# keillernogueira/dynamic-rs-segmentation

Hardware: AMD Instinct MI355X
Metric: training patches/sec dilated_grsl_rate8 64x64x5 (higher is better)
Workload: dtype f32; 1 GPU; dilated_grsl_rate8 (Dilated8Pooling) training step, single_fixed 64x64, 5-band synthetic 2048x2048 tile, global batch 128 (crop+augment+normalise, fwd, loss, bwd, momentum, confusion); global_batch=128, patch=64, bands=5, classes=6, parallelism=dp1, sync_bn=True, rccl_ranks_observed=1

## Files before the change

dynamic-rs-segmentation_amd/_lib.py:

```python
import ctypes as C
import os

_HERE = os.path.dirname(os.path.abspath(__file__))
LIB_PATH = os.path.join(_HERE, "libdrs_hip.so")
DEV_LIB_PATH = os.path.join(_HERE, "libdrs_hip_dev.so")

_p, _i, _f, _d = C.c_void_p, C.c_int, C.c_float, C.c_double
_sz, _u64 = C.c_size_t, C.c_ulonglong

SIGNATURES = {
    "drs_conv_mtile": (_i, [_i]),
    "drs_conv_forward": (_i, [_p, _i, _i, _i, _i, _i, _p, _p, _i, _i, _i, _i, _i, _p, _i, _i, _i, _p, _p]),
    "drs_conv_workspace_floats": (_sz, [_i]),
    "drs_conv_halo_skip": (_i, [_i, _i, _i, _i, _i, _i, _i]),
    "drs_conv_executed_ksteps": (_i, [_i, _i, _i, _i, _i, _i, _i, _p, _p]),
    "drs_conv_forward_ws": (_i, [_p, _i, _i, _i, _i, _i, _p, _p, _i, _i, _i, _i, _i, _p, _i, _i, _i, _p, _p, _sz, _p]),
    "drs_conv_wgrad_splits": (_i, [_i, _i, _i, _i, _i]),
    "drs_conv_wgrad": (_i, [_p, _i, _i, _i, _i, _i, _p, _i, _i, _i, _i, _i, _i, _i, _i, _i, _p, _p, _p]),
    "drs_filter_flip_transpose": (_i, [_p, _p, _i, _i, _i, _p]),
    "drs_filter_pad_cin": (_i, [_p, _p, _i, _i, _i, _i, _p]),
    "drs_split_conv_mtile": (_i, [_i]),
    "drs_split_terms": (_i, [_p, _sz, _i, _p, _p]),
    "drs_filter_split": (_i, [_p, _i, _i, _i, _i, _i, _p, _p, _p]),
    "drs_conv_forward_split": (_i, [_p, _i, _i, _i, _i, _i, _p, _p, _i, _i, _i, _i, _i, _p, _i, _i, _i, _p, _i, _p]),
    "drs_conv_wgrad_split_splits": (_i, [_i, _i, _i, _i, _i, _i, _i]),
    "drs_conv_wgrad_split": (_i, [_p, _i, _i, _i, _i, _i, _p, _i, _i, _i, _i, _i, _i, _i, _i, _i, _p, _p, _i, _p]),
    "drs_colsum_scratch_doubles": (_i, [_i]),
    "drs_stats_reduce": (_i, [_p, _i, _i, _p, _p, _p]),
    "drs_stats_reduce_means": (_i, [_p, _i, _i, _d, _p, _p, _p]),
    "drs_conv_stats_reduce": (_i, [_p, _i, _i, _i, _p, _p, _p]),
    "drs_conv_stats_finish": (_i, [_p, _i, _i, _i, _d, _p, _p, _p, _d, _i, _p, _p]),
    "drs_bn_finish": (_i, [_p, _d, _i, _p, _p, _p, _d, _i, _p]),
    "drs_bn_eval_coeffs": (_i, [_p, _p, _i, _p, _p]),
    "drs_bn_act_pool_forward": (_i, [_p, _i, _i, _i, _p, _f, _i, _p, _i, _i, _i, _p, _p]),
    "drs_bn_finish_act_pool_forward": (_i, [_p, _d, _p, _p, _p, _d, _i, _p, _i, _i, _i, _f, _i, _p, _i, _i, _i, _p, _p]),
    "drs_bn_act_pool_forward_terms": (_i, [_p, _i, _i, _i, _p, _f, _i, _p, _i, _i, _i, _p, _p, _i, _p]),
    "drs_bn_backward_rows": (_i, [_i, _i, _i, _i]),
    "drs_bn_backward_reduce": (_i, [_p, _i, _i, _p, _p, _i, _i, _i, _p, _f, _i, _p, _p, _p]),
    "drs_bn_backward_apply": (_i, [_p, _p, _i, _i, _i, _p, _p, _d, _p, _i, _i, _i, _p]),
    "drs_bn_backward_apply_means": (_i, [_p, _p, _i, _i, _i, _p, _p, _p, _i, _i, _i, _p]),
    "drs_bn_backward_apply_terms": (_i, [_p, _p, _i, _i, _i, _p, _p, _d, _p, _i, _i, _i, _p, _i, _p]),
    "drs_avg_pool_forward": (_i, [_p, _i, _i, _i, _i, _p, _i, _i, _i, _p]),
    "drs_avg_pool_backward": (_i, [_p, _i, _i, _i, _i, _i, _i, _p, _p]),
    "drs_se_forward": (_i, [_p, _i, _i, _i, _i, _p, _p, _p, _p, _p, _p, _p, _p, _i, _i, _i, _p]),
    "drs_se_backward": (_i, [_p, _i, _i, _p, _p, _p, _p, _p, _p, _i, _i, _i, _i, _p, _p, _p, _p, _p, _p, _p]),
    "drs_se_core_sums_scratch_doubles": (_i, [_i]),
    "drs_se_core_sums": (_i, [_p, _i, _i, _p, _i, _p, _p, _p]),
    "drs_se_gate": (_i, [_p, _d, _i, _i, _p, _p, _p, _p, _p, _p, _p, _p]),
    "drs_se_scale_const": (_i, [_p, _i, _i, _i, _p, _p, _i, _i, _i, _p]),
    "drs_classifier_rows": (_i, [_i, _i]),
    "drs_classifier_loss": (_i, [_p, _i, _i, _i, _i, _i, _i, _i, _p, _p, _p, _p, _p, _f, _p, _p, _p, _i, _i, _p, _p, _p,
                                 _p, _p]),
    "drs_classifier_loss_weighted": (_i, [_p, _i, _i, _i, _i, _i, _i, _i, _p, _p, _p, _p, _p, _f, _p, _p, _p, _p, _i, _i, _p, _p,
                                          _p, _p, _p]),
    "drs_classifier_loss_focal": (_i, [_p, _i, _i, _i, _i, _i, _i, _i, _p, _p, _p, _p, _p, _f, _p, _f, _p, _p, _p, _i, _i, _p, _p,
                                       _p, _p, _p]),
    "drs_label_histogram": (_i, [_p, _sz, _i, _i, _p, _p]),
    "drs_reliability_histogram": (_i, [_p, _p, _p, _sz, _i, _i, _p, _p]),
    "drs_temperature_scratch_doubles": (_sz, [_sz]),
    "drs_temperature_stats": (_i, [_p, _p, _p, _sz, _i, _i, _i, _d, _p, _p, _p]),
    "drs_rows_reduce_f32": (_i, [_p, _i, _i, _p, _p, _p]),
    "drs_sum_f64": (_i, [_p, _i, _p, _p]),
    "drs_l2_loss": (_i, [_p, _sz, _p, _p, _p]),
    "drs_momentum_update": (_i, [_p, _p, _p, _sz, _sz, _f, _f, _f, _f, _p]),
    "drs_confusion": (_i, [_p, _p, _p, _sz, _i, _i, _p, _p]),
    "drs_crop_normalize": (_i, [_p, _i, _p, _p, _p, _p, _p, _i, _p, _p, _p, _p, _p, _u64, _i, _p, _p, _i, _i, _i, _i, _p, _p,
                                _p, _i, _i, _p]),
    "drs_crop_normalize_scaled": (_i, [_p, _i, _p, _p, _p, _p, _p, _i, _i, _p, _p, _p, _p, _p, _p, _u64, _i, _p, _p, _i, _i, _i, _i,
                                       _p, _p, _p, _i, _i, _p]),
    "drs_stitch_accumulate": (_i, [_p, _p, _p, _i, _i, _i, _i, _i, _i, _i, _p]),
    "drs_stitch_finalize": (_i, [_p, _p, _i, _i, _i, _p, _p]),
    "drs_stitch_finalize_scores": (_i, [_p, _p, _i, _i, _i, _i, _p, _p, _p, _p, _p]),
    "drs_stitch_finalize_scores_t": (_i, [_p, _p, _i, _i, _i, _i, _f, _p, _p, _p, _p, _p]),
    "drs_tile_place": (_i, [_p, _p, _p, _i, _i, _i, _i, _p, _i, _p]),
    "drs_crop_dihedral": (_i, [_p, _i, _p, _p, _p, _i, _i, _p, _i, _p, _p, _i, _i, _i, _i, _p, _p]),
    "drs_tile_place_dihedral": (_i, [_p, _p, _p, _i, _i, _i, _i, _p, _i, _i, _p]),
    "drs_crop_resampled": (_i, [_p, _i, _p, _p, _p, _i, _i, _p, _i, _i, _i, _p, _p, _i, _i, _i, _i, _p, _p]),
    "drs_resample_accumulate": (_i, [_p, _p, _i, _i, _i, _i, _i, _i, _p, _p]),
    "drs_softmax_accumulate": (_i, [_p, _p, _i, _i, _i, _p, _p]),
    "drs_scale_f64": (_i, [_p, _i, _d, _p]),
    "drs_net_create": (_i, [C.c_char_p, _i, _i, _f, _i, _i, _i, _f, C.POINTER(_p)]),
    "drs_net_destroy": (None, [_p]),
    "drs_net_num_buffers": (_i, [_p]),
    "drs_net_buffer_info": (_i, [_p, _i, C.c_char_p, _i, C.POINTER(_sz), C.POINTER(_i)]),
    "drs_net_bind": (_i, [_p, C.c_char_p, _p, _sz]),
    "drs_net_buffer": (_i, [_p, C.c_char_p, C.POINTER(_p), C.POINTER(_sz)]),
    "drs_net_layout": (_i, [_p, C.POINTER(_sz), C.POINTER(_sz), C.POINTER(_sz), C.POINTER(_i), C.POINTER(_i), C.POINTER(_i)]),
    "drs_net_layer_info": (_i, [_p, _i, C.c_char_p, _i, C.POINTER(_i), C.c_char_p, C.c_char_p, _i, C.POINTER(_i), C.POINTER(_i)]),
    "drs_net_info": (_i, [_p, C.c_char_p, _i, C.POINTER(_f), C.POINTER(_i), C.c_char_p, _i, C.POINTER(_i), C.POINTER(_i)]),
    "drs_net_receptive_field": (_i, [_p, C.POINTER(_i), C.POINTER(_i)]),
    "drs_net_receptive_field_gated": (_i, [_p, C.POINTER(_i), C.POINTER(_i)]),
    "drs_net_se_info": (_i, [_p, _i, C.c_char_p, _i, C.POINTER(_i), C.POINTER(_i), C.POINTER(_i)]),
    "drs_net_type_name": (_i, [_i, C.c_char_p, _i, C.POINTER(_i)]),
    "drs_net_num_variables": (_i, [_p]),
    "drs_net_variable_info": (_i, [_p, _i, C.c_char_p, _i, C.POINTER(_sz), C.POINTER(_sz), C.POINTER(_i), C.POINTER(_i)]),
    "drs_params_get": (_i, [_p, C.c_char_p, C.c_char_p, _p, _sz, _p]),
    "drs_params_set": (_i, [_p, C.c_char_p, C.c_char_p, _p, _sz, _p]),
    "drs_grad_buffer": (_i, [_p, C.POINTER(_p), C.POINTER(_sz)]),
    "drs_net_global_step": (C.c_longlong, [_p, C.c_longlong]),
    "drs_net_learning_rate": (_f, [_p, _f]),
    "drs_net_set_comm": (_i, [_p, _i, _i, _p, _p, _p]),
    "drs_rccl_bind_library": (_i, [C.c_char_p]),
    "drs_rccl_available": (_i, []),
    "drs_rccl_form": (_i, []),
    "drs_rccl_unique_id": (_i, [_p]),
    "drs_rccl_comm_create": (_i, [_i, _i, _p, C.POINTER(_p)]),
    "drs_rccl_comm_destroy": (_i, [_p]),
    "drs_rccl_all_reduce": (_i, [_p, _p, C.c_size_t, _i, _p]),
    "drs_net_set_rccl": (_i, [_p, _i, _i, _p, _p, _p]),
    "drs_train_step": (_i, [_p, _i, _i, _f, _i, _d, _p]),
    "drs_forward": (_i, [_p, _i, _i, _i, _i, _p]),
    "drs_apply_update": (_i, [_p, _f, _p]),
    "drs_forward_staged": (_i, [_p, _i, _i, _i, _p, _i, _i, _p]),
    "drs_net_se_gate_finish": (_i, [_p, _i, _d, _p]),
    "drs_net_set_two_streams": (_i, [_p, _i]),
    "drs_net_set_class_weights": (_i, [_p, _p, _i]),
    "drs_net_get_class_weights": (_i, [_p, _p, _i, C.POINTER(_i)]),
    "drs_net_set_focal_gamma": (_i, [_p, _f]),
    "drs_net_get_focal_gamma": (_i, [_p, C.POINTER(_f)]),
    "drs_net_timing": (_i, [_p, _i]),
    "drs_net_num_timing_kinds": (_i, []),
    "drs_net_timing_summary": (_i, [_p, _i, C.c_char_p, _i, C.POINTER(_i), C.POINTER(_d), C.POINTER(_d)]),
}
ALLREDUCE_FN = C.CFUNCTYPE(_i, _p, _p, _sz, _i, _i, _p)
WAIT_FN = C.CFUNCTYPE(_i, _p, _i, _p)
WANT_LOGITS, WITH_LABELS, USE_ACC_MASK, USE_LOSS_MASK, NO_UPDATE = 1, 2, 4, 8, 16


DEV_SIGNATURES = {
    "drs_debug_skip_taps": (_i, [_i]), "drs_debug_conv_variant": (_i, [_i]), "drs_debug_conv_wide192": (_i, [_i]),
    "drs_debug_conv_splitk": (_i, [_i]), "drs_debug_conv_hybrid": (_i, [_i]), "drs_debug_conv_sk_order": (_i, [_i]), "drs_debug_conv_prio": (_i, [_i]),
    "drs_debug_conv_sk_geometry": (_i, [_i, _i, _i, _p]), "drs_debug_conv_trace": (_i, [_p]), "drs_debug_conv_lpt": (_i, [_i]), "drs_debug_conv_order": (_i, [_i] * 7 + [_p, _i]),
    "drs_debug_conv_image_tiles": (_i, [_i]), "drs_debug_conv_order_image": (_i, [_i] * 7 + [_p, _i]),
    "drs_debug_wgrad_variant": (_i, [_i]), "drs_debug_wgrad_seg": (_i, [_i]), "drs_debug_wgrad_balance": (_i, [_i]), "drs_debug_wgrad_target": (_i, [_i]),
    "drs_debug_wgrad_target_big": (_i, [_i]), "drs_debug_wgrad_len": (_i, [_i]), "drs_debug_wgrad_minchunks": (_i, [_i]), "drs_debug_wgrad_model": (_i, [_i]), "drs_debug_wgrad_ablate": (_i, [_i]), "drs_debug_wgrad_prio": (_i, [_i]), "drs_debug_cls_variant": (_i, [_i]), "drs_debug_slide_blocks": (_i, [_i]), "drs_debug_slide_minrows": (_i, [_i]), "drs_debug_slide_rowpad": (_i, [_i]), "drs_debug_chain_mode": (_i, [_i]), "drs_debug_jitter": (_i, [C.c_ulonglong]), "drs_debug_wg_stream_prio": (_i, [_i]), "drs_debug_reductions_on_chain": (_i, [_i]), "drs_debug_wgrad_schedule": (_i, [_i, _i, _i]), "drs_debug_variant": (_i, [_i]),
    "drs_debug_wgrad_cut": (_i, [_i] * 7 + [_p, _i, _p, _p]),
}


class DrsError(RuntimeError):
    pass


_lib = None
_dev = None


def _open(path, signatures):
    if not os.path.isfile(path):
        raise DrsError("HIP library not built: %s is missing (run dynamic-rs-segmentation_amd/csrc/build.sh "
                       "or __graft_entry__.build()); there is no CPU fallback" % path)
    import torch
    lib = C.CDLL(path)
    for name, (res, args) in signatures.items():
        fn = getattr(lib, name)
        fn.restype = res
        fn.argtypes = args
    return lib


def load():
    global _lib
    if _lib is None:
        _lib = _open(LIB_PATH, SIGNATURES)
    return _lib


class _Dev(object):

    def __init__(self, lib):
        self.lib = lib

    def __getattr__(self, name):
        return getattr(self.lib, name)

    def load(self):
        return self.lib

    def call(self, name, *args):
        rc = getattr(self.lib, name)(*args)
        if rc != 0:
            raise DrsError("%s -> %s" % (name, _STATUS.get(rc, rc)))

    def query(self, name, *args):
        return getattr(self.lib, name)(*args)


def dev():
    global _dev
    if _dev is None:
        sig = dict(SIGNATURES)
        sig.update(DEV_SIGNATURES)
        _dev = _Dev(_open(DEV_LIB_PATH, sig))
    return _dev


_STATUS = {1: "DRS_ERR_ARG (rejected argument)", 2: "DRS_ERR_HIP (launch failed)"}


def call(name, *args):
    rc = getattr(load(), name)(*args)
    if rc != 0:
        raise DrsError("%s -> %s" % (name, _STATUS.get(rc, rc)))


def query(name, *args):
    return getattr(load(), name)(*args)
```

dynamic-rs-segmentation_amd/csrc/conv_mfma.hip:

```cpp
#include "drs_common.hpp"
#include <algorithm>
#include <cstdlib>
#include <map>
#include <mutex>
#include <numeric>
#include <tuple>
#include <vector>

namespace {

constexpr int BK = 32;
constexpr int LDA = BK + 4;

struct ConvArgs {
  const float* in; int S, P, ld_in, coff_in;
  int M;
  const float* w;
  const float* bias;
  float* out; int ld_out, coff_out;
  float* stats;
  int k, rate, pad, Cin, Cout;
  int accumulate;
  int skip_halo;
  float rcpS, rcpSS;
  float* sk_slab;
  int sk_W, sk_nks, sk_U;
  int sk_T, sk_tiles, sk_G, sk_order;
  int prio;
  int lpt_T, lpt_ta, lpt_tb, lpt_P;
  int img_g;
  const int* img_order;
#ifdef DRS_DEV
  unsigned long long* trace;
#endif
};

__device__ __forceinline__ void set_prio_by_progress(int done, int total, int& quarter, int mode = 1) {
  const int q = __builtin_amdgcn_readfirstlane((done * 4) / total);
  if (q == quarter) return;
  quarter = q;
  if (mode == 2) {
    if (q <= 0) __builtin_amdgcn_s_setprio(2);
    else if (q == 1) __builtin_amdgcn_s_setprio(1);
    else __builtin_amdgcn_s_setprio(0);
    return;
  }
  if (q <= 0) __builtin_amdgcn_s_setprio(3);
  else if (q == 1) __builtin_amdgcn_s_setprio(2);
  else if (q == 2) __builtin_amdgcn_s_setprio(1);
  else __builtin_amdgcn_s_setprio(0);
}

__host__ __device__ __forceinline__ int lpt_tile(int wg, int T, int ta, int tb, int P, int ntn) {
  const int per = P * T * ntn, nI = tb - ta, nE = T - nI;
  const int chunk = wg / per;
  int wl = wg - chunk * per, p, t;
  if (wl < P * nI * ntn) {
    p = wl / (nI * ntn);
    wl -= p * nI * ntn;
    t = ta + wl / ntn;
  } else {
    wl -= P * nI * ntn;
    p = wl / (nE * ntn);
    wl -= p * nE * ntn;
    const int e = wl / ntn;
    t = e < ta ? e : tb + (e - ta);
  }
  return ((chunk * P + p) * T + t) * ntn + wl % ntn;
}

__host__ __device__ __forceinline__ int sk_first_unit(int w, int U, int W) { return (int)((long long)w * U / W); }
__host__ __device__ __forceinline__ int sk_owner(int x, int U, int W) { return (int)((((long long)x + 1) * W - 1) / U); }

template <int BM, int BN, int WM, int WN, bool MAP = false>
__device__ __forceinline__ void conv_epilogue(const ConvArgs& a, f32x16 (&acc)[BM / WM / 32][BN / WN / 32], float* scratch, int m0, int n0,
                                              int pix0 = 0, int pcs = 30) {
  constexpr int WTM = BM / WM, WTN = BN / WN;
  constexpr int TM = WTM / 32, TN = WTN / 32;
  const int t = threadIdx.x;
  const int lane = t & 63, wave = t >> 6;
  const int li = lane & 31, h = lane >> 5;
  const int wm = wave / WN, wn = wave % WN;
  const int pcm = (1 << pcs) - 1, S2 = a.S * a.S;
  const int lane_rl = wm * WTM + 4 * h;
  const int lane_pix = MAP ? pix0 + (lane_rl >> pcs) * S2 + (lane_rl & pcm) : 0;
  float bv[TN];
#pragma unroll
  for (int ni = 0; ni < TN; ++ni) {
    const int col = n0 + wn * WTN + ni * 32 + li;
    bv[ni] = a.bias ? a.bias[col] : 0.f;
#pragma unroll
    for (int mi = 0; mi < TM; ++mi) {
#pragma unroll
      for (int r = 0; r < 16; ++r) {
        const int crl = mi * 32 + (r & 3) + 8 * (r >> 2);
        const int row = MAP ? lane_pix + __builtin_amdgcn_readfirstlane((crl >> pcs) * S2 + (crl & pcm)) : m0 + lane_rl + crl;
        if (row < a.M) {
          float v = acc[mi][ni][r] + bv[ni];
          float* dst = a.out + (size_t)row * a.ld_out + a.coff_out + col;
          if (a.accumulate) v += *dst;
          *dst = v;
        }
      }
    }
  }
  if (a.stats) {
    const int rem = a.M - m0;
    tile_column_stats<TN, WM, BN>(
        scratch, t, wm, h == 0, (float)(rem < BM ? rem : BM), [&](int ni) { return wn * WTN + ni * 32 + li; },
        [](float s) { return s + __shfl_xor(s, 32); },
        [&](int ni, auto f) {
#pragma unroll
          for (int mi = 0; mi < TM; ++mi)
#pragma unroll
            for (int r = 0; r < 16; ++r)
              if (m0 + wm * WTM + mi * 32 + (r & 3) + 8 * (r >> 2) + 4 * h < a.M) f(acc[mi][ni][r] + bv[ni]);
        },
        a.stats + ((size_t)(m0 / BM) * a.Cout + n0) * 2);
  }
}

template <int BM, int BN, int WM, int WN, bool PACK = false>
__global__ __launch_bounds__(256, (BM == 256 || BN == 128) ? 3 : 1) void conv_igemm_kernel(const ConvArgs a) {
  static_assert(WM * WN == 4, "4 waves");
  constexpr int LDB = BN + 4;
  constexpr int WTM = BM / WM, WTN = BN / WN;
  constexpr int TM = WTM / 32, TN = WTN / 32;
  constexpr int NA = BM / 32;
  constexpr int NB = BN / 32;
  constexpr int BROWS = 256 / (BN / 4);

  __shared__ __attribute__((aligned(16))) float lds[BM * LDA + BK * LDB];
  float* As = lds;
  float* Bs = lds + BM * LDA;

  const int t = threadIdx.x;
  const int lane = t & 63, wave = t >> 6;
  const int li = lane & 31, h = lane >> 5;
  const int wm = wave / WN, wn = wave % WN;

  const int ntn = a.Cout / BN;
  const int nblk = gridDim.x;
  const int tile = xcd_remap(blockIdx.x, nblk);
  const int m0 = (tile / ntn) * BM;
  const int n0 = (tile % ntn) * BN;

  const int Sp = a.S + 2 * a.P;
  uint32_t offA[NA];
#pragma unroll
  for (int i = 0; i < NA; ++i) {
    int p = m0 + (t >> 3) + 32 * i;
    p = p < a.M ? p : a.M - 1;
    offA[i] = (padded_pixel_off(p, a.S, a.P, a.ld_in, a.rcpS, a.rcpSS, -a.pad, -a.pad) + (uint32_t)(a.coff_in + (PACK ? 0 : (t & 7) * 4))) * 4u;
  }
  const int brow = t / (BN / 4), bcol = (t % (BN / 4)) * 4;
  uint32_t offB[NB];
#pragma unroll
  for (int i = 0; i < NB; ++i) offB[i] = (uint32_t)((brow + BROWS * i) * a.Cout + n0 + bcol) * 4u;

  f32x16 acc[TM][TN];
#pragma unroll
  for (int mi = 0; mi < TM; ++mi)
#pragma unroll
    for (int ni = 0; ni < TN; ++ni)
#pragma unroll
      for (int r = 0; r < 16; ++r) acc[mi][ni][r] = 0.f;

  const int cpt = a.Cin / BK;
  int u_lo, u_hi;
  live_tap_rows(m0, BM, a.M, a.S, a.k, a.rate, a.pad, a.rcpS, a.rcpSS, u_lo, u_hi);
  if (PACK || !a.skip_halo) { u_lo = 0; u_hi = a.k; }
  u_lo = __builtin_amdgcn_readfirstlane(u_lo);
  u_hi = __builtin_amdgcn_readfirstlane(u_hi);
  const int nks = PACK ? (a.k * a.k * a.Cin + BK - 1) / BK : (u_hi - u_lo) * a.k * cpt;
  const char* wlive = reinterpret_cast<const char*>(a.w + (size_t)u_lo * a.k * a.Cin * a.Cout);
  const char* inb = reinterpret_cast<const char*>(a.in);
  f32x4 ra[NA], rb[NB];
  int lu = u_lo, lv = 0, lc = 0;

  auto gload = [&](int ks) {
    if (PACK) {
      const int kidx = ks * BK + (t & 7) * 4;
      int tap = kidx / a.Cin;
      const int c = kidx - tap * a.Cin;
      tap = tap < a.k * a.k ? tap : a.k * a.k - 1;
      const int u = tap / a.k, v = tap - u * a.k;
      const uint32_t soff = (uint32_t)((u * a.rate * Sp + v * a.rate) * a.ld_in + c) * 4u;
#pragma unroll
      for (int i = 0; i < NA; ++i) ra[i] = *reinterpret_cast<const f32x4*>(inb + (offA[i] + soff));
    } else {
      const char* ab = inb + (size_t)(uint32_t)((lu * a.rate * Sp + lv * a.rate) * a.ld_in + lc * BK) * 4u;
#pragma unroll
      for (int i = 0; i < NA; ++i) { uint32_t o = offA[i]; asm volatile("" : "+v"(o)); ra[i] = *reinterpret_cast<const f32x4*>(ab + o); }
    }
    const char* wb = wlive + (size_t)(uint32_t)((PACK ? ks : ((lu - u_lo) * a.k + lv) * cpt + lc) * BK) * (uint32_t)a.Cout * 4u;
#pragma unroll
    for (int i = 0; i < NB; ++i) { uint32_t o = offB[i]; asm volatile("" : "+v"(o)); rb[i] = *reinterpret_cast<const f32x4*>(wb + o); }
    if (!PACK) { if (++lv == a.k) { lv = 0; if (++lu == u_hi) { lu = u_lo; ++lc; } } }
  };
  auto lstore = [&]() {
#pragma unroll
    for (int i = 0; i < NA; ++i) *reinterpret_cast<f32x4*>(&As[((t >> 3) + 32 * i) * LDA + (t & 7) * 4]) = ra[i];
#pragma unroll
    for (int i = 0; i < NB; ++i) *reinterpret_cast<f32x4*>(&Bs[(brow + BROWS * i) * LDB + bcol]) = rb[i];
  };

  gload(0);
  lstore();
  __syncthreads();
  const int arow = wm * WTM + li, bcolw = wn * WTN + li;
  for (int ks = 0; ks < nks; ++ks) {
    if (ks + 1 < nks) gload(ks + 1);
    {
      constexpr int NST = BK / 2;
      f32x4 af[2][TM];
      float bf[2][TN];
#pragma unroll
      for (int mi = 0; mi < TM; ++mi) af[0][mi] = *reinterpret_cast<const f32x4*>(&As[(arow + mi * 32) * LDA + h * 4]);
#pragma unroll
      for (int ni = 0; ni < TN; ++ni) bf[0][ni] = Bs[(h * 4) * LDB + bcolw + ni * 32];
#pragma unroll
      for (int st = 0; st < NST; ++st) {
        const int e = st & 3;
        if (st + 1 < NST) {
          const int q1 = (st + 1) >> 2, e1 = (st + 1) & 3;
#pragma unroll
          for (int ni = 0; ni < TN; ++ni) bf[(st + 1) & 1][ni] = Bs[(q1 * 8 + h * 4 + e1) * LDB + bcolw + ni * 32];
          if (e1 == 0) {
#pragma unroll
            for (int mi = 0; mi < TM; ++mi) af[q1 & 1][mi] = *reinterpret_cast<const f32x4*>(&As[(arow + mi * 32) * LDA + q1 * 8 + h * 4]);
            __builtin_amdgcn_sched_group_barrier(0x100, TN + TM, 0);
          } else {
            __builtin_amdgcn_sched_group_barrier(0x100, TN, 0);
          }
        }
#pragma unroll
        for (int mi = 0; mi < TM; ++mi)
#pragma unroll
          for (int ni = 0; ni < TN; ++ni)
            acc[mi][ni] = __builtin_amdgcn_mfma_f32_32x32x2f32(af[(st >> 2) & 1][mi][e], bf[st & 1][ni], acc[mi][ni], 0, 0, 0);
        __builtin_amdgcn_sched_group_barrier(0x8, TM * TN, 0);
      }
    }
    __syncthreads();
    if (ks + 1 < nks) { lstore(); __syncthreads(); }
  }

  conv_epilogue<BM, BN, WM, WN>(a, acc, lds, m0, n0);
}

template <int BM, int BN, int WM, int WN, bool SK>
__global__ __launch_bounds__(256, 3) void conv_dma_kernel(const ConvArgs a) {
#if defined(__HIP_DEVICE_COMPILE__)
  static_assert(WM * WN == 4 && BM == 128, "4 waves, 128-pixel tiles");
  constexpr int WTM = BM / WM, WTN = BN / WN;
  constexpr int TM = WTM / 32, TN = WTN / 32;
  constexpr int HK = 16;
  constexpr int ASTAGE = BM * HK, STAGE = ASTAGE + HK * BN;
  constexpr int IA = (BM / 16) / 4;
  constexpr int BQ = BN / 4;
  constexpr int IB = HK * BQ / 64 / 4;
  static_assert(IA >= 1 && IB >= 1 && IB * 4 * 64 == HK * BQ, "tile / wave layout");

  __shared__ __attribute__((aligned(1024))) float lds[2 * STAGE];

  const int t = threadIdx.x;
  const int lane = t & 63, wave = __builtin_amdgcn_readfirstlane(t >> 6);
  const int li = lane & 31, h = lane >> 5;
  const int wm = wave / WN, wn = wave % WN;
  const int ntn = a.Cout / BN;
  const int wg = xcd_remap(blockIdx.x, gridDim.x);
#ifdef DRS_DEV
  if (a.trace && t == 0) a.trace[2 * blockIdx.x] = __builtin_amdgcn_s_memrealtime();
#endif
  const int Sp = a.S + 2 * a.P;
  const int cpt = a.Cin / BK;
  typedef __attribute__((address_space(3))) void* lds_ptr;
  const __amdgpu_buffer_rsrc_t rsrc_in = __builtin_amdgcn_make_buffer_rsrc(const_cast<float*>(a.in), 0, 0xffffffff, 0x00020000);
  const __amdgpu_buffer_rsrc_t rsrc_w = __builtin_amdgcn_make_buffer_rsrc(const_cast<float*>(a.w), 0, 0xffffffff, 0x00020000);
  const int arow = wm * WTM + li, bcolw = wn * WTN + li;
  const int sw = (li >> 2) & 3;

  int u = 0, u_end = 1, rng = 0, dp_next = 0;
  bool dp_first = false;
  if (SK) {
    const int jb = (int)(((long long)wg * a.sk_W + a.sk_G - 1) / a.sk_G), je = (int)(((long long)(wg + 1) * a.sk_W + a.sk_G - 1) / a.sk_G);
    rng = __builtin_amdgcn_readfirstlane(jb);
    u = u_end = 0;
    if (je > jb) {
      u = __builtin_amdgcn_readfirstlane(sk_first_unit(jb, a.sk_U, a.sk_W));
      u_end = __builtin_amdgcn_readfirstlane(sk_first_unit(jb + 1, a.sk_U, a.sk_W));
    }
    dp_next = a.sk_T + wg;
    if (u >= u_end && dp_next >= a.sk_tiles) return;
    dp_first = a.sk_order == 1 || (a.sk_order == 2 && ((blockIdx.x >> 8) & 1));
  }
  const int img_g = SK ? 0 : a.img_g;
  int tile0 = wg;
  if (!SK && img_g) {
    const int mpos = wg / ntn;
    tile0 = __builtin_amdgcn_readfirstlane(a.img_order[mpos] * ntn + (wg - mpos * ntn));
  } else if (!SK && a.lpt_T) {
    tile0 = __builtin_amdgcn_readfirstlane(lpt_tile(wg, a.lpt_T, a.lpt_ta, a.lpt_tb, a.lpt_P, ntn));
  }
  bool first_seg = true;
  int quart = -1, done = 0, total = 1;
  if (a.prio == 3) __builtin_amdgcn_s_setprio(3);
  if (SK && a.prio) total = (u_end - u) + (dp_next < a.sk_tiles ? ((a.sk_tiles - 1 - dp_next) / a.sk_G + 1) * a.sk_nks : 0);
  for (;;) {
    int tile = tile0, kb = 0, ke = 0;
    bool in_range = false;
    if (SK) {
      in_range = u < u_end && !(dp_first && dp_next < a.sk_tiles);
      if (in_range) {
        tile = u / a.sk_nks;
        kb = u - tile * a.sk_nks;
        ke = kb + (u_end - u);
        ke = ke < a.sk_nks ? ke : a.sk_nks;
      } else {
        tile = dp_next;
        dp_next += a.sk_G;
        kb = 0;
        ke = a.sk_nks;
      }
    }
    const int m0 = (tile / ntn) * BM;
    const int n0 = (tile % ntn) * BN;
    int ty = 0, tx0 = 0, timg0 = 0;
    if (!SK && img_g) {
      const int grp = image_tile_pos(tile / ntn, a.S, img_g, ty, tx0);
      ty = __builtin_amdgcn_readfirstlane(ty);
      tx0 = __builtin_amdgcn_readfirstlane(tx0);
      timg0 = __builtin_amdgcn_readfirstlane(grp << img_g);
    }

    uint32_t offA[IA], offB[IB];
#pragma unroll
    for (int i = 0; i < IA; ++i) {
      const int r = (wave + 4 * i) * 16 + (lane >> 2);
      uint32_t pix;
      if (!SK && img_g) {
        const int pcs = 7 - img_g;
        pix = (uint32_t)(((timg0 + (r >> pcs)) * Sp + ty + a.P - a.pad) * Sp + (tx0 + (r & ((1 << pcs) - 1)) + a.P - a.pad)) * (uint32_t)a.ld_in;
      } else {
        int p = m0 + r;
        p = p < a.M ? p : a.M - 1;
        pix = padded_pixel_off(p, a.S, a.P, a.ld_in, a.rcpS, a.rcpSS, -a.pad, -a.pad);
      }
      offA[i] = (pix + (uint32_t)a.coff_in) * 4u + (uint32_t)(((lane & 3) ^ ((lane >> 4) & 3)) * 16);
    }
#pragma unroll
    for (int i = 0; i < IB; ++i) {
      const int f = 64 * (wave + 4 * i) + lane;
      offB[i] = (uint32_t)(((f / BQ) * a.Cout + n0 + (f % BQ) * 4)) * 4u;
    }

    f32x16 acc[TM][TN];
#pragma unroll
    for (int mi = 0; mi < TM; ++mi)
#pragma unroll
      for (int ni = 0; ni < TN; ++ni)
#pragma unroll
        for (int r = 0; r < 16; ++r) acc[mi][ni][r] = 0.f;

    int u_lo, u_hi, v_lo = 0, v_hi = a.k;
    if (!SK && img_g) live_taps_image_tile(ty, tx0, 128 >> img_g, a.S, a.k, a.rate, a.pad, u_lo, u_hi, v_lo, v_hi);
    else live_tap_rows(m0, BM, a.M, a.S, a.k, a.rate, a.pad, a.rcpS, a.rcpSS, u_lo, u_hi);
    if (!a.skip_halo || SK) { u_lo = 0; u_hi = a.k; v_lo = 0; v_hi = a.k; }
    u_lo = __builtin_amdgcn_readfirstlane(u_lo);
    u_hi = __builtin_amdgcn_readfirstlane(u_hi);
    v_lo = __builtin_amdgcn_readfirstlane(v_lo);
    v_hi = __builtin_amdgcn_readfirstlane(v_hi);
    const int nks = (u_hi - u_lo) * (v_hi - v_lo) * cpt;
    if (!SK) ke = nks;
    const uint32_t wlive_off = (uint32_t)(u_lo * a.k * a.Cin * a.Cout) * 4u;
    int lu = u_lo, lv = v_lo, lc = 0;
    if (SK && kb) {
      const int per_chunk = (u_hi - u_lo) * a.k;
      lc = kb / per_chunk;
      const int rem = kb - lc * per_chunk;
      lu = u_lo + rem / a.k;
      lv = rem - (rem / a.k) * a.k;
      lc = __builtin_amdgcn_readfirstlane(lc); lu = __builtin_amdgcn_readfirstlane(lu); lv = __builtin_amdgcn_readfirstlane(lv);
    }

    auto issue = [&](int half, int stage) {
      float* sa = lds + stage * STAGE;
      float* sb = sa + ASTAGE;
      const uint32_t ao = (uint32_t)((lu * a.rate * Sp + lv * a.rate) * a.ld_in + lc * BK + half * HK) * 4u;
      const uint32_t wo = wlive_off + (uint32_t)((((lu - u_lo) * a.k + lv) * cpt + lc) * BK + half * HK) * (uint32_t)a.Cout * 4u;
#pragma unroll
      for (int i = 0; i < IA; ++i)
        __builtin_amdgcn_raw_ptr_buffer_load_lds(rsrc_in, (lds_ptr)(sa + (wave + 4 * i) * 256), 16, (int)offA[i], (int)ao, 0, 0);
#pragma unroll
      for (int i = 0; i < IB; ++i)
        __builtin_amdgcn_raw_ptr_buffer_load_lds(rsrc_w, (lds_ptr)(sb + (wave + 4 * i) * 256), 16, (int)offB[i], (int)wo, 0, 0);
    };
    auto next_kstep = [&]() { if (++lv == v_hi) { lv = v_lo; if (++lu == u_hi) { lu = u_lo; ++lc; } } };

    auto compute = [&](int stage) {
      const float* As = lds + stage * STAGE;
      const float* Bs = As + ASTAGE;
      constexpr int NST = HK / 2;
      f32x4 af[2][TM];
      float bf[2][TN];
#pragma unroll
      for (int mi = 0; mi < TM; ++mi) af[0][mi] = *reinterpret_cast<const f32x4*>(&As[(arow + mi * 32) * HK + ((h ^ sw) * 4)]);
#pragma unroll
      for (int ni = 0; ni < TN; ++ni) bf[0][ni] = Bs[(h * 4) * BN + bcolw + ni * 32];
#pragma unroll
      for (int st = 0; st < NST; ++st) {
        const int e = st & 3;
        if (st + 1 < NST) {
          const int q1 = (st + 1) >> 2, e1 = (st + 1) & 3;
#pragma unroll
          for (int ni = 0; ni < TN; ++ni) bf[(st + 1) & 1][ni] = Bs[(q1 * 8 + h * 4 + e1) * BN + bcolw + ni * 32];
          if (e1 == 0) {
#pragma unroll
            for (int mi = 0; mi < TM; ++mi)
              af[q1 & 1][mi] = *reinterpret_cast<const f32x4*>(&As[(arow + mi * 32) * HK + (((2 * q1 + h) ^ sw) * 4)]);
            __builtin_amdgcn_sched_group_barrier(0x100, TN + TM, 0);
          } else {
            __builtin_amdgcn_sched_group_barrier(0x100, TN, 0);
          }
        }
#pragma unroll
        for (int mi = 0; mi < TM; ++mi)
#pragma unroll
          for (int ni = 0; ni < TN; ++ni)
            acc[mi][ni] = __builtin_amdgcn_mfma_f32_32x32x2f32(af[(st >> 2) & 1][mi][e], bf[st & 1][ni], acc[mi][ni], 0, 0, 0);
        __builtin_amdgcn_sched_group_barrier(0x8, TM * TN, 0);
      }
    };

    issue(0, 0);
    asm volatile("s_waitcnt vmcnt(0)" ::: "memory");
    __syncthreads();
    if (!SK && a.prio) total = nks;
    for (int ks = kb; ks < ke; ++ks) {
      if (a.prio == 1) set_prio_by_progress(SK ? done + (ks - kb) : ks, total, quart);
      issue(1, 1);
      compute(0);
      asm volatile("s_waitcnt vmcnt(0)" ::: "memory");
      __syncthreads();
      next_kstep();
      if (ks + 1 < ke) issue(0, 0);
      compute(1);
      asm volatile("s_waitcnt vmcnt(0)" ::: "memory");
      __syncthreads();
    }
    if (!SK) {
      conv_epilogue<BM, BN, WM, WN, true>(a, acc, lds, m0, n0, img_g ? (timg0 * a.S + ty) * a.S + tx0 : m0, img_g ? 7 - img_g : 30);
    } else if (kb == 0 && ke == nks) {
      conv_epilogue<BM, BN, WM, WN>(a, acc, lds, m0, n0);
    } else {
      float* piece = a.sk_slab + (size_t)(2 * rng + (first_seg ? 0 : 1)) * (BM * BN) + (size_t)wave * (TM * TN * 16 * 64) + lane * 4;
#pragma unroll
      for (int mi = 0; mi < TM; ++mi)
#pragma unroll
        for (int ni = 0; ni < TN; ++ni)
#pragma unroll
          for (int q = 0; q < 4; ++q)
            *reinterpret_cast<f32x4*>(piece + ((mi * TN + ni) * 4 + q) * 256) =
                f32x4{acc[mi][ni][4 * q], acc[mi][ni][4 * q + 1], acc[mi][ni][4 * q + 2], acc[mi][ni][4 * q + 3]};
    }
    if (!SK) break;
    done += ke - kb;
    if (in_range) { u += ke - kb; first_seg = false; }
    if (u >= u_end && dp_next >= a.sk_tiles) break;
    __syncthreads();
  }
#ifdef DRS_DEV
  if (a.trace && t == 0) a.trace[2 * blockIdx.x + 1] = __builtin_amdgcn_s_memrealtime();
#endif
#endif
}

template <int BM, int BN, int WM, int WN>
__global__ __launch_bounds__(256) void conv_sk_fixup_kernel(const ConvArgs a) {
  constexpr int WTM = BM / WM, WTN = BN / WN;
  constexpr int TM = WTM / 32, TN = WTN / 32;
  __shared__ float lds[2 * WM * BN];
  if (a.prio == 3) __builtin_amdgcn_s_setprio(3);
  const int tile = blockIdx.x;
  const int x0 = tile * a.sk_nks;
  const int w_first = sk_owner(x0, a.sk_U, a.sk_W), w_last = sk_owner(x0 + a.sk_nks - 1, a.sk_U, a.sk_W);
  if (w_first == w_last) return;
  const int lane = threadIdx.x & 63, wave = threadIdx.x >> 6;
  const int ntn = a.Cout / BN;
  const int m0 = (tile / ntn) * BM, n0 = (tile % ntn) * BN;
  f32x16 acc[TM][TN];
#pragma unroll
  for (int mi = 0; mi < TM; ++mi)
#pragma unroll
    for (int ni = 0; ni < TN; ++ni)
#pragma unroll
      for (int r = 0; r < 16; ++r) acc[mi][ni][r] = 0.f;
  auto piece_of = [&](int w) {
    const int slot = 2 * w + (sk_first_unit(w, a.sk_U, a.sk_W) >= x0 ? 0 : 1);
    return a.sk_slab + (size_t)slot * (BM * BN) + (size_t)wave * (TM * TN * 16 * 64) + lane * 4;
  };
  constexpr int NF = TM * TN * 4;
  int w = w_first;
  if (NF <= 16) {
    for (; w + 1 <= w_last; w += 2) {
      const float* pa = piece_of(w);
      const float* pb = piece_of(w + 1);
      f32x4 va[NF], vb[NF];
#pragma unroll
      for (int f = 0; f < NF; ++f) va[f] = *reinterpret_cast<const f32x4*>(pa + f * 256);
#pragma unroll
      for (int f = 0; f < NF; ++f) vb[f] = *reinterpret_cast<const f32x4*>(pb + f * 256);
#pragma unroll
      for (int f = 0; f < NF; ++f)
#pragma unroll
        for (int j = 0; j < 4; ++j) acc[(f >> 2) / TN][(f >> 2) % TN][4 * (f & 3) + j] += va[f][j];
#pragma unroll
      for (int f = 0; f < NF; ++f)
#pragma unroll
        for (int j = 0; j < 4; ++j) acc[(f >> 2) / TN][(f >> 2) % TN][4 * (f & 3) + j] += vb[f][j];
    }
  }
  for (; w <= w_last; ++w) {
    const float* piece = piece_of(w);
#pragma unroll
    for (int mi = 0; mi < TM; ++mi)
#pragma unroll
      for (int ni = 0; ni < TN; ++ni)
#pragma unroll
        for (int q = 0; q < 4; ++q) {
          const f32x4 v = *reinterpret_cast<const f32x4*>(piece + ((mi * TN + ni) * 4 + q) * 256);
#pragma unroll
          for (int j = 0; j < 4; ++j) acc[mi][ni][4 * q + j] += v[j];
        }
  }
  conv_epilogue<BM, BN, WM, WN>(a, acc, lds, m0, n0);
}

constexpr int WG_MAXT = 64, WG_MAXC = 8;
struct WgradPlan {
  int nclass;
  int n[WG_MAXC];
  int seg_start[WG_MAXC + 1];
  int seg_width[WG_MAXC];
  unsigned char cls[WG_MAXT];
};

struct WgradArgs {
  const float* x; int S, Px, ld_x, coff_x;
  const float* g; int Pg, ld_g, coff_g;
  int M;
  int k, rate, pad, Cin, Cout;
  float* slab;
  int chunks_per_split;
  int ntr, nto;
  int skip_halo;
  int live_cut;
  int prio;
  int ablate;
  float rcpS, rcpSS;
  WgradPlan plan;
#ifdef DRS_DEV
  unsigned long long* trace;
#endif
};

__host__ __device__ __forceinline__ int wave_uniform(int v) {
#if defined(__HIP_DEVICE_COMPILE__)
  return __builtin_amdgcn_readfirstlane(v);
#else
  return v;
#endif
}

__host__ __device__ __forceinline__ void wgrad_assign(const WgradArgs& a, int TR, int id, int& tile, int& split, int& cbeg, int& cend,
                                                      int& live_lo, int& live_hi) {
  const int nchunks_total = (a.M + 31) / 32;
  const int rows_all = a.k * a.k * a.Cin;
  int nr = 0;
  if (a.plan.nclass == 0) {
    const int ntile = a.ntr * a.nto;
    split = id / ntile;
    tile = id % ntile;
  } else {
    int j = 0;
    while (j + 1 < a.plan.nclass && id >= a.plan.seg_start[j + 1]) ++j;
    const int rel = id - a.plan.seg_start[j];
    split = (j ? a.plan.n[j - 1] : 0) + rel / a.plan.seg_width[j];
    const int pos = rel % a.plan.seg_width[j];
    const int want = pos / a.nto;
    int r = 0, seen = 0;
    for (; r < a.ntr; ++r)
      if (a.plan.cls[r] >= j) { if (seen == want) break; ++seen; }
    r = r < a.ntr ? r : a.ntr - 1;
    tile = r * a.nto + pos % a.nto;
    nr = a.plan.n[a.plan.cls[r]];
  }
  tile = wave_uniform(tile);
  split = wave_uniform(split);
  const int R0 = (tile / a.nto) * TR;
  const int rlast = (R0 + TR < rows_all ? R0 + TR : rows_all) - 1;
  int lo, hi;
  live_pixel_range(R0, rlast, a.Cin, a.k, a.rate, a.pad, a.S, a.live_cut, lo, hi);
  if (a.plan.nclass == 0) {
    cbeg = split * a.chunks_per_split;
    cend = cbeg + a.chunks_per_split;
    cend = cend < nchunks_total ? cend : nchunks_total;
  } else {
    const int S2 = a.S * a.S, lp = hi - lo;
    const int live_total = (a.M / S2) * lp;
    const int q = (live_total + nr - 1) / nr;
    auto bound = [&](int s) -> int {
      if (s <= 0) return 0;
      const long long jp = (long long)s * q;
      if (s >= nr || jp >= live_total) return nchunks_total;
      const int img = (int)jp / lp, rem = (int)jp - img * lp;
      return (img * S2 + lo + rem) >> 5;
    };
    cbeg = bound(split);
    cend = bound(split + 1);
  }
  cbeg = wave_uniform(cbeg);
  cend = wave_uniform(cend);
  if (!a.skip_halo) { lo = 0; hi = a.S * a.S; }
  live_lo = lo; live_hi = hi;
}

struct ChunkWalk {
  int c, b, r, y, x0;
  int S, S2, lo, hi, ylo;
  __device__ __forceinline__ void init(int cfirst, int S_, float rcpS, float rcpSS, int lo_, int hi_) {
    S = S_; S2 = S_ * S_; lo = lo_; hi = hi_;
    int q;
    divmod24(lo, S, rcpS, ylo, q);
    c = next_live_chunk(cfirst - 1, S2, rcpSS, lo, hi);
    divmod24(c * 32, S2, rcpSS, b, r);
    divmod24(r, S, rcpS, y, x0);
    c = __builtin_amdgcn_readfirstlane(c); b = __builtin_amdgcn_readfirstlane(b); r = __builtin_amdgcn_readfirstlane(r);
    y = __builtin_amdgcn_readfirstlane(y); x0 = __builtin_amdgcn_readfirstlane(x0); ylo = __builtin_amdgcn_readfirstlane(ylo);
  }
  __device__ __forceinline__ int advance() {
    int r1 = r + 32, b1 = b;
    if (r1 >= S2) { r1 -= S2; ++b1; }
    if ((r1 + 31 >= lo && r1 < hi) || r1 + 31 >= S2 + lo) {
      ++c; r = r1; b = b1;
      x0 += 32;
      if (x0 >= S) { x0 -= S; ++y; }
      if (y >= S) y = 0;
      return 1;
    }
    const int tb = r1 < lo ? b1 : b1 + 1;
    const int T = tb * S2 + lo, c_old = c;
    const int f = T & 31;
    c = T >> 5;
    if (f <= lo) { b = tb; r = lo - f; } else { b = tb - 1; r = S2 + lo - f; }
    if (f == 0) { y = ylo; x0 = 0; } else { x0 = S - f; y = ylo - 1; if (y < 0) y = S - 1; }
    return c - c_old;
  }
};

template <int TR, int TO, bool AFF>
__global__ __launch_bounds__(64 * (TR >= 64 ? 2 : 1) * (TO >= 64 ? 2 : 1), 3) void wgrad_kernel(const WgradArgs a) {
  constexpr int WR = TR >= 64 ? 2 : 1, WC = TO >= 64 ? 2 : 1;
  constexpr int NT = 64 * WR * WC;
  constexpr int WTR = TR / WR, WTO = TO / WC;
  constexpr int TMr = WTR / 32, TNo = WTO / 32;
  constexpr int BP = 32;
  constexpr int LDX = TR + 4, LDG = TO + 4;
  constexpr int XQ = TR / 4, GQ = TO / 4;
  constexpr int NX = BP * XQ / NT, NG = BP * GQ / NT;
  constexpr int XPS = NT / XQ, GPS = NT / GQ;

  __shared__ __attribute__((aligned(16))) float lds[BP * LDX + BP * LDG];
  __shared__ uint32_t tabx[2][BP], tabg[2][BP];
  float* Xs = lds;
  float* Gs = lds + BP * LDX;

  const int t = threadIdx.x;
  const int lane = t & 63, wave = t >> 6;
  const int li = lane & 31, h = lane >> 5;
  const int wr = wave / WC, wc = wave % WC;

  int tile, split, cbeg, cend, live_lo, live_hi;
#ifdef DRS_DEV
  if (a.trace && t == 0) {
    a.trace[2 * blockIdx.x] = __builtin_amdgcn_s_memrealtime();
    a.trace[32768 + blockIdx.x] = (unsigned long long)__builtin_amdgcn_s_getreg(63492) | ((unsigned long long)__builtin_amdgcn_s_getreg(63508) << 32);
  }
#endif
  wgrad_assign(a, TR, xcd_remap(blockIdx.x, gridDim.x), tile, split, cbeg, cend, live_lo, live_hi);
  const int R0 = (tile / a.nto) * TR;
  const int o0 = (tile % a.nto) * TO;
  const int rows_all = a.k * a.k * a.Cin;
  const int myR = R0 + (t % XQ) * 4;
  const int myRc = myR < rows_all ? myR : 0;
  const int tap = myRc / a.Cin, c0 = myRc % a.Cin;
  const int u = tap / a.k, v = tap % a.k;
  const int Sxp = a.S + 2 * a.Px, Sgp = a.S + 2 * a.Pg;
  const uint32_t xconst = (uint32_t)((u * a.rate * Sxp + v * a.rate) * a.ld_x + a.coff_x + c0) * 4u;
  const uint32_t gconst = (uint32_t)(a.coff_g + o0 + (t % GQ) * 4) * 4u;
  const int xpix = t / XQ, gpix = t / GQ;
  constexpr bool affine = AFF;
  uint32_t xoff[NX], goff[NG];
#pragma unroll
  for (int i = 0; i < NX; ++i) xoff[i] = xconst + (affine ? (uint32_t)((xpix + XPS * i) * a.ld_x) * 4u : 0u);
#pragma unroll
  for (int i = 0; i < NG; ++i) goff[i] = gconst + (affine ? (uint32_t)((gpix + GPS * i) * a.ld_g) * 4u : 0u);

  f32x16 acc[TMr][TNo];
#pragma unroll
  for (int mi = 0; mi < TMr; ++mi)
#pragma unroll
    for (int ni = 0; ni < TNo; ++ni)
#pragma unroll
      for (int r = 0; r < 16; ++r) acc[mi][ni][r] = 0.f;

  const int nchunks_total = (a.M + BP - 1) / BP;
  const int clast = (a.M & 31) ? nchunks_total - 1 : -1;
  ChunkWalk w;
  w.init(cbeg, a.S, a.rcpS, a.rcpSS, live_lo, live_hi);

  int py = 0, px = 0;
  uint32_t ox = 0, og = 0;
  const uint32_t stepx = (uint32_t)(32 * a.ld_x) * 4u, stepg = (uint32_t)(32 * a.ld_g) * 4u;
  const uint32_t rowjx = (uint32_t)((Sxp - a.S) * a.ld_x) * 4u, rowjg = (uint32_t)((Sgp - a.S) * a.ld_g) * 4u;
  const uint32_t imgjx = (uint32_t)(Sxp * (Sxp - a.S) * a.ld_x) * 4u, imgjg = (uint32_t)(Sgp * (Sgp - a.S) * a.ld_g) * 4u;
  auto pixel_from_index = [&](int p) {
    int pb, rem;
    divmod24(p < a.M ? p : a.M - 1, w.S2, a.rcpSS, pb, rem);
    divmod24(rem, a.S, a.rcpS, py, px);
    ox = (uint32_t)(((pb * Sxp + py + a.Px - a.pad) * Sxp + px + a.Px - a.pad) * a.ld_x) * 4u;
    og = (uint32_t)(((pb * Sgp + py + a.Pg) * Sgp + px + a.Pg) * a.ld_g) * 4u;
  };
  if (!affine && t < BP) pixel_from_index(w.c * BP + t);
  auto fill_tables = [&](int slot, int stepped) {
    if (affine || t >= BP || w.c >= cend) return;
    const int p = w.c * BP + t;
    if (stepped == 1 && p < a.M && a.S >= 11) {
      px += 32; ox += stepx; og += stepg;
      if (a.S >= 32) {
        if (px >= a.S) { px -= a.S; ++py; ox += rowjx; og += rowjg; }
      } else {
#pragma unroll
        for (int k = 0; k < 3; ++k) if (px >= a.S) { px -= a.S; ++py; ox += rowjx; og += rowjg; }
      }
      if (py >= a.S) { py -= a.S; ox += imgjx; og += imgjg; }
    } else if (stepped != 0) {
      pixel_from_index(p);
    }
    tabx[slot][t] = ox;
    tabg[slot][t] = og;
  };

  const char* xbase = reinterpret_cast<const char*>(a.x);
  const char* gbase = reinterpret_cast<const char*>(a.g);
  f32x4 rx[NX], rg[NG];
  uint32_t nox[NX], nog[NG];
#pragma unroll
  for (int i = 0; i < NX; ++i) nox[i] = 0u;
#pragma unroll
  for (int i = 0; i < NG; ++i) nog[i] = 0u;
  auto fetch_offsets = [&](int slot) {
    if (affine) return;
#pragma unroll
    for (int i = 0; i < NX; ++i) nox[i] = tabx[slot][xpix + XPS * i] + xoff[i];
#pragma unroll
    for (int i = 0; i < NG; ++i) nog[i] = tabg[slot][gpix + GPS * i] + goff[i];
  };
  auto gload = [&]() {
    if (affine) {
      const char* xb = xbase + (size_t)(uint32_t)(((w.b * Sxp + w.y + a.Px - a.pad) * Sxp + w.x0 + a.Px - a.pad) * a.ld_x) * 4u;
      const char* gb = gbase + (size_t)(uint32_t)(((w.b * Sgp + w.y + a.Pg) * Sgp + w.x0 + a.Pg) * a.ld_g) * 4u;
#pragma unroll
      for (int i = 0; i < NX; ++i) { uint32_t o = xoff[i]; asm volatile("" : "+v"(o)); rx[i] = *reinterpret_cast<const f32x4*>(xb + o); }
#pragma unroll
      for (int i = 0; i < NG; ++i) { uint32_t o = goff[i]; asm volatile("" : "+v"(o)); rg[i] = *reinterpret_cast<const f32x4*>(gb + o); }
    } else {
#pragma unroll
      for (int i = 0; i < NX; ++i) rx[i] = *reinterpret_cast<const f32x4*>(xbase + nox[i]);
#pragma unroll
      for (int i = 0; i < NG; ++i) rg[i] = *reinterpret_cast<const f32x4*>(gbase + nog[i]);
    }
  };
  auto lstore = [&](int chunk) {
#pragma unroll
    for (int i = 0; i < NX; ++i) *reinterpret_cast<f32x4*>(&Xs[(xpix + XPS * i) * LDX + (t % XQ) * 4]) = rx[i];
    if (!AFF && chunk == clast) {
#pragma unroll
      for (int i = 0; i < NG; ++i)
        *reinterpret_cast<f32x4*>(&Gs[(gpix + GPS * i) * LDG + (t % GQ) * 4]) =
            chunk * BP + gpix + GPS * i < a.M ? rg[i] : f32x4{0.f, 0.f, 0.f, 0.f};
    } else {
#pragma unroll
      for (int i = 0; i < NG; ++i) *reinterpret_cast<f32x4*>(&Gs[(gpix + GPS * i) * LDG + (t % GQ) * 4]) = rg[i];
    }
  };

  int cA = w.c;
  if (cA < cend) {
    fill_tables(0, 0);
    __syncthreads();
    fetch_offsets(0);
    gload();
    int stepped = w.advance();
    int cB = w.c;
    fill_tables(1, stepped);
    lstore(cA);
    __syncthreads();
    fetch_offsets(1);
    const int xr = wr * WTR + li, gc = wc * WTO + li;
    int quart = -1;
    for (int it = 0; cA < cend; ++it) {
      if (a.prio) set_prio_by_progress(cA - cbeg, cend - cbeg, quart, a.prio);
#ifdef DRS_DEV
      if (a.ablate == 2) fetch_offsets((it + 1) & 1);
#endif
      if (cB < cend) gload();
      stepped = w.advance();
      fill_tables(it & 1, stepped);
      {
        float af[2][TMr], bf[2][TNo];
#pragma unroll
        for (int mi = 0; mi < TMr; ++mi) af[0][mi] = Xs[h * LDX + xr + mi * 32];
#pragma unroll
        for (int ni = 0; ni < TNo; ++ni) bf[0][ni] = Gs[h * LDG + gc + ni * 32];
#pragma unroll
        for (int s = 0; s < BP / 2; ++s) {
          if (s + 1 < BP / 2) {
#pragma unroll
            for (int mi = 0; mi < TMr; ++mi) af[(s + 1) & 1][mi] = Xs[(2 * s + 2 + h) * LDX + xr + mi * 32];
#pragma unroll
            for (int ni = 0; ni < TNo; ++ni) bf[(s + 1) & 1][ni] = Gs[(2 * s + 2 + h) * LDG + gc + ni * 32];
            __builtin_amdgcn_sched_group_barrier(0x100, TMr + TNo, 0);
          }
#pragma unroll
          for (int mi = 0; mi < TMr; ++mi)
#pragma unroll
            for (int ni = 0; ni < TNo; ++ni)
              acc[mi][ni] = __builtin_amdgcn_mfma_f32_32x32x2f32(af[s & 1][mi], bf[s & 1][ni], acc[mi][ni], 0, 0, 0);
          __builtin_amdgcn_sched_group_barrier(0x8, TMr * TNo, 0);
        }
      }
      __syncthreads();
      fetch_offsets(it & 1);
      if (cB < cend) { lstore(cB); __syncthreads(); }
      cA = cB;
      cB = w.c;
    }
  }
  const size_t rows_total = (size_t)a.k * a.k * a.Cin;
  float* dst = a.slab + ((size_t)split * rows_total + R0) * a.Cout + o0;
#pragma unroll
  for (int mi = 0; mi < TMr; ++mi)
#pragma unroll
    for (int ni = 0; ni < TNo; ++ni)
#pragma unroll
      for (int r = 0; r < 16; ++r) {
        const int row = wr * WTR + mi * 32 + (r & 3) + 8 * (r >> 2) + 4 * h;
        const int col = wc * WTO + ni * 32 + li;
        if (R0 + row < rows_all) dst[(size_t)row * a.Cout + col] = acc[mi][ni][r];
      }
#ifdef DRS_DEV
  if (a.trace && t == 0) a.trace[2 * blockIdx.x + 1] = __builtin_amdgcn_s_memrealtime();
#endif
}

template <int TR, int TO, int MODE>
__global__ __launch_bounds__(64 * (TR >= 64 ? 2 : 1) * (TO >= 64 ? 2 : 1), 3) void wgrad_dma_kernel(const WgradArgs a) {
#if defined(__HIP_DEVICE_COMPILE__)
  constexpr int WR = TR >= 64 ? 2 : 1, WC = TO >= 64 ? 2 : 1;
  constexpr int NW = WR * WC, NT = 64 * NW;
  constexpr int WTR = TR / WR, WTO = TO / WC;
  constexpr int TMr = WTR / 32, TNo = WTO / 32;
  constexpr int BP = 32, HP = 16;
  constexpr int XQ = TR / 4, GQ = TO / 4;
  constexpr int IX = HP * XQ / 64 / NW, IG = HP * GQ / 64 / NW;
  static_assert(IX >= 1 && IG >= 1 && IX * NW * 64 == HP * XQ && IG * NW * 64 == HP * GQ, "tile / wave layout");
  constexpr int XSTAGE = HP * TR, STAGE = HP * (TR + TO);

  __shared__ __attribute__((aligned(1024))) float lds[2 * STAGE];
  __shared__ uint32_t tabx[2][BP], tabg[2][BP];

  constexpr bool AFF = MODE == 1;
  constexpr bool SEG = MODE == 2;
  const int t = threadIdx.x;
  const int lane = t & 63, wave = (AFF || SEG) ? __builtin_amdgcn_readfirstlane(t >> 6) : t >> 6;
  const int li = lane & 31, h = lane >> 5;
  const int wr = wave / WC, wc = wave % WC;

  int tile, split, cbeg, cend, live_lo, live_hi;
#ifdef DRS_DEV
  if (a.trace && t == 0) {
    a.trace[2 * blockIdx.x] = __builtin_amdgcn_s_memrealtime();
    a.trace[32768 + blockIdx.x] = (unsigned long long)__builtin_amdgcn_s_getreg(63492) | ((unsigned long long)__builtin_amdgcn_s_getreg(63508) << 32);
  }
#endif
  wgrad_assign(a, TR, xcd_remap(blockIdx.x, gridDim.x), tile, split, cbeg, cend, live_lo, live_hi);
  const int R0 = (tile / a.nto) * TR;
  const int o0 = (tile % a.nto) * TO;
  const int rows_all = a.k * a.k * a.Cin;
  const int Sxp = a.S + 2 * a.Px, Sgp = a.S + 2 * a.Pg;
  constexpr bool affine = AFF || SEG;
  const int xq = lane % XQ;
  const int myR = R0 + xq * 4;
  const int myRc = myR < rows_all ? myR : 0;
  const int tap = myRc / a.Cin, c0 = myRc % a.Cin;
  const int u = tap / a.k, v = tap % a.k;
  const uint32_t biasx = SEG ? (uint32_t)(32 * a.ld_x) * 4u : 0u, biasg = SEG ? (uint32_t)(32 * a.ld_g) * 4u : 0u;
  const uint32_t xconst = (uint32_t)((a.ablate == 1 ? 0 : (u * a.rate * Sxp + v * a.rate)) * a.ld_x + a.coff_x + c0) * 4u + biasx;
  uint32_t xoff[IX], goff[IG];
  int xpix[IX], gpix[IG];
#pragma unroll
  for (int i = 0; i < IX; ++i) {
    xpix[i] = (64 * (wave + NW * i) + lane) / XQ;
    xoff[i] = xconst + (affine ? (uint32_t)(xpix[i] * a.ld_x) * 4u : 0u);
  }
#pragma unroll
  for (int i = 0; i < IG; ++i) {
    const int f = 64 * (wave + NW * i) + lane;
    gpix[i] = f / GQ;
    goff[i] = (uint32_t)(a.coff_g + o0 + (f % GQ) * 4) * 4u + (affine ? (uint32_t)(gpix[i] * a.ld_g) * 4u : 0u) + biasg;
  }

  f32x16 acc[TMr][TNo];
#pragma unroll
  for (int mi = 0; mi < TMr; ++mi)
#pragma unroll
    for (int ni = 0; ni < TNo; ++ni)
#pragma unroll
      for (int r = 0; r < 16; ++r) acc[mi][ni][r] = 0.f;

  const int nchunks_total = (a.M + BP - 1) / BP;
  const int clast = (a.M & 31) ? nchunks_total - 1 : -1;
  ChunkWalk w;
  w.init(cbeg, a.S, a.rcpS, a.rcpSS, live_lo, live_hi);

  int py = 0, px = 0;
  uint32_t ox = 0, og = 0;
  const uint32_t stepx = (uint32_t)(32 * a.ld_x) * 4u, stepg = (uint32_t)(32 * a.ld_g) * 4u;
  const uint32_t rowjx = (uint32_t)((Sxp - a.S) * a.ld_x) * 4u, rowjg = (uint32_t)((Sgp - a.S) * a.ld_g) * 4u;
  const uint32_t imgjx = (uint32_t)(Sxp * (Sxp - a.S) * a.ld_x) * 4u, imgjg = (uint32_t)(Sgp * (Sgp - a.S) * a.ld_g) * 4u;
  auto pixel_from_index = [&](int p) {
    int pb, rem;
    divmod24(p < a.M ? p : a.M - 1, w.S2, a.rcpSS, pb, rem);
    divmod24(rem, a.S, a.rcpS, py, px);
    ox = (uint32_t)(((pb * Sxp + py + a.Px - a.pad) * Sxp + px + a.Px - a.pad) * a.ld_x) * 4u;
    og = (uint32_t)(((pb * Sgp + py + a.Pg) * Sgp + px + a.Pg) * a.ld_g) * 4u;
  };
  if (!affine && t < BP) pixel_from_index(w.c * BP + t);
  auto fill_tables = [&](int slot, int stepped) {
    if (affine || t >= BP || w.c >= cend) return;
    const int p = w.c * BP + t;
    if (stepped == 1 && p < a.M && a.S >= 11) {
      px += 32; ox += stepx; og += stepg;
      if (a.S >= 32) {
        if (px >= a.S) { px -= a.S; ++py; ox += rowjx; og += rowjg; }
      } else {
#pragma unroll
        for (int k = 0; k < 3; ++k) if (px >= a.S) { px -= a.S; ++py; ox += rowjx; og += rowjg; }
      }
      if (py >= a.S) { py -= a.S; ox += imgjx; og += imgjg; }
    } else if (stepped != 0) {
      pixel_from_index(p);
    }
    tabx[slot][t] = ox;
    tabg[slot][t] = og;
  };

  const char* xbase = reinterpret_cast<const char*>(a.x);
  const char* gbase = reinterpret_cast<const char*>(a.g);
  typedef __attribute__((address_space(3))) void* lds_ptr;
  struct Seg { int brk; int32_t jx, jg; };
  auto chunk_bases = [&](const char*& xb, const char*& gb, Seg& sg) {
    xb = xbase + (size_t)(uint32_t)(((w.b * Sxp + w.y + a.Px - a.pad) * Sxp + w.x0 + a.Px - a.pad) * a.ld_x) * 4u;
    gb = gbase + (size_t)(uint32_t)(((w.b * Sgp + w.y + a.Pg) * Sgp + w.x0 + a.Pg) * a.ld_g) * 4u;
    if (SEG) {
      xb -= biasx; gb -= biasg;
      sg.brk = a.S - w.x0;
      const bool last = w.c == clast, img_end = w.y == a.S - 1;
      sg.jx = last ? -(int32_t)biasx : (int32_t)(rowjx + (img_end ? imgjx : 0u));
      sg.jg = last ? -(int32_t)biasg : (int32_t)(rowjg + (img_end ? imgjg : 0u));
    }
  };
  struct LaneOffsets { uint32_t x[2][IX], g[2][IG]; };
  auto fetch_offsets = [&](int slot, LaneOffsets& o) {
    if (affine) return;
#pragma unroll
    for (int half = 0; half < 2; ++half) {
#pragma unroll
      for (int i = 0; i < IX; ++i) o.x[half][i] = tabx[slot][half * HP + xpix[i]] + xoff[i];
#pragma unroll
      for (int i = 0; i < IG; ++i) o.g[half][i] = tabg[slot][half * HP + gpix[i]] + goff[i];
    }
  };
  auto issue = [&](const char* xb, const char* gb, const Seg& seg, const LaneOffsets& o, int half, int stage) {
    float* sx = lds + stage * STAGE;
    float* sg = sx + XSTAGE;
    if (affine) {
      const char* xh = xb + (size_t)(uint32_t)(half * HP * a.ld_x) * 4u;
      const char* gh = gb + (size_t)(uint32_t)(half * HP * a.ld_g) * 4u;
      int inner = HP;
      if (SEG) {
        const int hb = seg.brk - half * HP;
        if (hb <= 0) { xh += (ptrdiff_t)seg.jx; gh += (ptrdiff_t)seg.jg; }
        else if (hb < HP) inner = hb;
      }
      if (SEG && inner < HP) {
#pragma unroll
        for (int i = 0; i < IX; ++i) {
          uint32_t v = xoff[i] + (xpix[i] >= inner ? (uint32_t)seg.jx : 0u);
          __builtin_amdgcn_global_load_lds(xh + v, (lds_ptr)(sx + (wave + NW * i) * 256), 16, 0, 0);
        }
#pragma unroll
        for (int i = 0; i < IG; ++i) {
          uint32_t v = goff[i] + (gpix[i] >= inner ? (uint32_t)seg.jg : 0u);
          __builtin_amdgcn_global_load_lds(gh + v, (lds_ptr)(sg + (wave + NW * i) * 256), 16, 0, 0);
        }
      } else {
#pragma unroll
        for (int i = 0; i < IX; ++i) {
          uint32_t v = xoff[i]; asm volatile("" : "+v"(v));
          __builtin_amdgcn_global_load_lds(xh + v, (lds_ptr)(sx + (wave + NW * i) * 256), 16, 0, 0);
        }
#pragma unroll
        for (int i = 0; i < IG; ++i) {
          uint32_t v = goff[i]; asm volatile("" : "+v"(v));
          __builtin_amdgcn_global_load_lds(gh + v, (lds_ptr)(sg + (wave + NW * i) * 256), 16, 0, 0);
        }
      }
    } else {
#pragma unroll
      for (int i = 0; i < IX; ++i) __builtin_amdgcn_global_load_lds(xbase + o.x[half][i], (lds_ptr)(sx + (wave + NW * i) * 256), 16, 0, 0);
#pragma unroll
      for (int i = 0; i < IG; ++i) __builtin_amdgcn_global_load_lds(gbase + o.g[half][i], (lds_ptr)(sg + (wave + NW * i) * 256), 16, 0, 0);
    }
  };
  auto zero_tail = [&](int chunk, int half, int stage) {
    if (AFF || chunk != clast) return;
    float* sg = lds + stage * STAGE + XSTAGE;
    for (int e = t; e < HP * TO; e += NT)
      if (chunk * BP + half * HP + e / TO >= a.M) sg[e] = 0.f;
    __syncthreads();
  };
  const int xr = wr * 32 + li, gc = wc * 32 + li;
  constexpr int XG = 32 * WR, GG = 32 * WC;
  auto compute = [&](int stage) {
    const float* Xs = lds + stage * STAGE;
    const float* Gs = Xs + XSTAGE;
    float af[2][TMr], bf[2][TNo];
#pragma unroll
    for (int mi = 0; mi < TMr; ++mi) af[0][mi] = Xs[h * TR + xr + mi * XG];
#pragma unroll
    for (int ni = 0; ni < TNo; ++ni) bf[0][ni] = Gs[h * TO + gc + ni * GG];
#pragma unroll
    for (int s = 0; s < HP / 2; ++s) {
      if (s + 1 < HP / 2) {
#pragma unroll
        for (int mi = 0; mi < TMr; ++mi) af[(s + 1) & 1][mi] = Xs[(2 * s + 2 + h) * TR + xr + mi * XG];
#pragma unroll
        for (int ni = 0; ni < TNo; ++ni) bf[(s + 1) & 1][ni] = Gs[(2 * s + 2 + h) * TO + gc + ni * GG];
        __builtin_amdgcn_sched_group_barrier(0x100, TMr + TNo, 0);
      }
#pragma unroll
      for (int mi = 0; mi < TMr; ++mi)
#pragma unroll
        for (int ni = 0; ni < TNo; ++ni)
          acc[mi][ni] = __builtin_amdgcn_mfma_f32_32x32x2f32(af[s & 1][mi], bf[s & 1][ni], acc[mi][ni], 0, 0, 0);
      __builtin_amdgcn_sched_group_barrier(0x8, TMr * TNo, 0);
    }
  };

  int cA = w.c;
  if (cA < cend) {
    const char *xbA, *gbA, *xbB = xbase, *gbB = gbase;
    LaneOffsets oA, oB;
#pragma unroll
    for (int half = 0; half < 2; ++half) {
#pragma unroll
      for (int i = 0; i < IX; ++i) oA.x[half][i] = oB.x[half][i] = 0u;
#pragma unroll
      for (int i = 0; i < IG; ++i) oA.g[half][i] = oB.g[half][i] = 0u;
    }
    Seg sgA = {32, 0, 0}, sgB = {32, 0, 0};
    chunk_bases(xbA, gbA, sgA);
    fill_tables(0, 0);
    if (!affine) __syncthreads();
    fetch_offsets(0, oA);
    issue(xbA, gbA, sgA, oA, 0, 0);
    int stepped = w.advance();
    int cB = w.c;
    chunk_bases(xbB, gbB, sgB);
    fill_tables(1, stepped);
    asm volatile("s_waitcnt vmcnt(0)" ::: "memory");
    __syncthreads();
    zero_tail(cA, 0, 0);
    int quart = -1;
    for (int it = 0; cA < cend; ++it) {
      if (a.prio) set_prio_by_progress(cA - cbeg, cend - cbeg, quart, a.prio);
#ifdef DRS_DEV
      const bool late = a.ablate == 2;
      if (late) fetch_offsets(it & 1, oA); else
#endif
      fetch_offsets((it + 1) & 1, oB);
      issue(xbA, gbA, sgA, oA, 1, 1);
      compute(0);
      asm volatile("s_waitcnt vmcnt(0)" ::: "memory");
      __syncthreads();
      zero_tail(cA, 1, 1);
#ifdef DRS_DEV
      if (late) fetch_offsets((it + 1) & 1, oB);
#endif
      if (cB < cend) issue(xbB, gbB, sgB, oB, 0, 0);
      stepped = w.advance();
      compute(1);
      fill_tables(it & 1, stepped);
      asm volatile("s_waitcnt vmcnt(0)" ::: "memory");
      __syncthreads();
      if (cB < cend) zero_tail(cB, 0, 0);
      cA = cB; xbA = xbB; gbA = gbB; sgA = sgB;
      oA = oB;
      cB = w.c;
      chunk_bases(xbB, gbB, sgB);
    }
  }
  const size_t rows_total = (size_t)a.k * a.k * a.Cin;
  float* dst = a.slab + ((size_t)split * rows_total + R0) * a.Cout + o0;
#pragma unroll
  for (int mi = 0; mi < TMr; ++mi)
#pragma unroll
    for (int ni = 0; ni < TNo; ++ni)
#pragma unroll
      for (int r = 0; r < 16; ++r) {
        const int row = mi * XG + wr * 32 + (r & 3) + 8 * (r >> 2) + 4 * h;
        const int col = ni * GG + wc * 32 + li;
        if (R0 + row < rows_all) dst[(size_t)row * a.Cout + col] = acc[mi][ni][r];
      }
#ifdef DRS_DEV
  if (a.trace && t == 0) a.trace[2 * blockIdx.x + 1] = __builtin_amdgcn_s_memrealtime();
#endif
#endif
}

__global__ void wgrad_reduce_kernel(const float* __restrict__ slab, float* __restrict__ grad, int nsplit_all, int taps,
                                    int cin_pad, int cin_real, int cout, int tr, const WgradPlan plan) {
  const int n = taps * cin_real * cout;
  for (int i = blockIdx.x * blockDim.x + threadIdx.x; i < n; i += gridDim.x * blockDim.x) {
    const int o = i % cout;
    const int rc = i / cout;
    const int c = rc % cin_real, tap = rc / cin_real;
    const size_t src = ((size_t)tap * cin_pad + c) * cout + o;
    const int nsplit = plan.nclass ? plan.n[plan.cls[(tap * cin_pad + c) / tr]] : nsplit_all;
    const size_t stride = (size_t)taps * cin_pad * cout;
    float s = 0.f;
    int k = 0;
    for (; k + 8 <= nsplit; k += 8) {
      float v[8];
#pragma unroll
      for (int j = 0; j < 8; ++j) v[j] = slab[(size_t)(k + j) * stride + src];
#pragma unroll
      for (int j = 0; j < 8; ++j) s += v[j];
    }
    for (; k < nsplit; ++k) s += slab[(size_t)k * stride + src];
    grad[i] = s;
  }
}

__global__ void flip_transpose_kernel(const float* __restrict__ w, float* __restrict__ wt, int k, int cin, int cout) {
  const int n = k * k * cin * cout;
  for (int i = blockIdx.x * blockDim.x + threadIdx.x; i < n; i += gridDim.x * blockDim.x) {
    const int c = i % cin;
    int rest = i / cin;
    const int o = rest % cout;
    rest /= cout;
    const int v = rest % k, u = rest / k;
    wt[i] = w[(((k - 1 - u) * k + (k - 1 - v)) * cin + c) * cout + o];
  }
}

__global__ void step_prep_kernel(const StepPrepArgs a) {
  const int e = blockIdx.y;
  const int i0 = blockIdx.x * blockDim.x + threadIdx.x, stride = gridDim.x * blockDim.x;
  if (e < a.n) {
    const int k = a.k[e], cin = a.cin[e], cout = a.cout[e];
    const float* __restrict__ w = a.w[e];
    float* __restrict__ wt = a.wt[e];
    const int n = k * k * cin * cout;
    for (int i = i0; i < n; i += stride) {
      const int c = i % cin;
      int rest = i / cin;
      const int o = rest % cout;
      rest /= cout;
      const int v = rest % k, u = rest / k;
      wt[i] = w[(((k - 1 - u) * k + (k - 1 - v)) * cin + c) * cout + o];
    }
  } else if (e == a.n) {
    for (int i = i0; i < a.nz0; i += stride) a.z0[i] = 0u;
  } else {
    for (int i = i0; i < a.nz1; i += stride) a.z1[i] = 0.f;
  }
}

__global__ void pad_cin_kernel(const float* __restrict__ w, float* __restrict__ wp, int taps, int cin, int cin_pad, int cout) {
  const int n = taps * cin_pad * cout;
  for (int i = blockIdx.x * blockDim.x + threadIdx.x; i < n; i += gridDim.x * blockDim.x) {
    const int o = i % cout;
    const int rc = i / cout;
    const int c = rc % cin_pad, tap = rc / cin_pad;
    wp[i] = c < cin ? w[((size_t)tap * cin + c) * cout + o] : 0.f;
  }
}

int g_conv_variant = -1;

#ifdef DRS_DEV
unsigned long long* g_conv_trace = nullptr;
#endif
int g_conv_lpt = 1;
int g_conv_splitk = -1;
int g_conv_sk_order = 1;
int g_conv_prio = -1;

constexpr int SK_MAX_TILES = 4096;

int cu_count() {
  static int cached[64];
  int dev = 0;
  if (hipGetDevice(&dev) != hipSuccess || dev < 0 || dev >= 64) return 256;
  if (cached[dev] == 0) {
    hipDeviceProp_t p;
    cached[dev] = (hipGetDeviceProperties(&p, dev) == hipSuccess && p.multiProcessorCount >= 1) ? p.multiProcessorCount : 256;
  }
  return cached[dev];
}
inline int sk_max_w() { return 3 * cu_count(); }

struct SkGeom { int G, W, T; };
int g_conv_hybrid = 1;
SkGeom sk_geometry(int tiles, int nks, int bn, size_t ws_floats) {
  const SkGeom plain = {0, 0, 0};
  if (g_conv_splitk == 0 || tiles >= SK_MAX_TILES || nks < 2) return plain;
  const long long NCU = cu_count();
  long long cap = (long long)(ws_floats / (2ull * 128 * (size_t)bn));
  if (cap > sk_max_w()) cap = sk_max_w();
  if (cap < 1) return plain;
  const int MINU = 12;
  const int occ = 3;
  long long G, W, T = tiles;
  if (g_conv_splitk > 0) {
    G = W = g_conv_splitk;
  } else {
    const long long per = (tiles + NCU - 1) / NCU;
    if ((double)tiles >= 0.93 * (double)NCU * (double)per) return plain;
    const long long U = (long long)tiles * nks;
    long long per_cu = U / (NCU * MINU);
    per_cu = per_cu < 1 ? 1 : (per_cu > occ ? occ : per_cu);
    G = W = NCU * per_cu;
    if (U < NCU * MINU) G = W = U / MINU > 0 ? U / MINU : 1;
  }
  if (g_conv_hybrid && tiles > G) {
    T = tiles % G;
    if (T == 0) return plain;
    W = G;
  }
  if (W > T * nks) W = T * nks;
  if (W > G) W = G;
  if (W > cap) {
    if (g_conv_splitk <= 0) return plain;
    W = cap; if (G < W || T == tiles) G = W;
  }
  return SkGeom{(int)G, (int)W, (int)T};
}

void conv_lpt_setup(ConvArgs& a, int BM, int mt, int nt, int W) {
  a.lpt_T = 0; a.lpt_ta = a.lpt_tb = a.lpt_P = 0;
  if (W || !g_conv_lpt || drs_g_skip_halo_taps == 0) return;
  const int S2 = a.S * a.S, T = S2 % BM == 0 ? S2 / BM : 0, nblk = mt * nt;
  if (T < 2 || BM % a.S != 0 || nblk % 8 != 0 || (nblk / 8) % (T * nt) != 0) return;
  const int rows = BM / a.S;
  auto full = [&](int t) {
    const int y0 = t * rows, y1 = y0 + rows - 1;
    const int lo = a.pad - y1 > 0 ? (a.pad - y1 + a.rate - 1) / a.rate : 0;
    int hi = (a.S - 1 - y0 + a.pad) / a.rate + 1;
    hi = hi < a.k ? hi : a.k;
    return lo == 0 && hi == a.k;
  };
  int ta = 0, tb = T;
  while (ta < T && !full(ta)) ++ta;
  while (tb > ta && !full(tb - 1)) --tb;
  bool ok = ta < tb;
  for (int t = ta; ok && t < tb; ++t) ok = full(t);
  if (ok && (ta > 0 || tb < T)) { a.lpt_T = T; a.lpt_ta = ta; a.lpt_tb = tb; a.lpt_P = nblk / 8 / (T * nt); a.skip_halo = 1; }
}

int g_conv_image_tiles = -1;

int conv_image_tiles_rule(int k, int rate, int cin, int cout, int B, int S) {
  if (B != 128 || S != 64) return 0;
  struct Row { int k, rate, cin, cout; };
  static const Row gains[] = {{4, 3, 64, 128},
                              {4, 4, 128, 128},
                              {3, 5, 128, 192}, {3, 5, 192, 128},
                              {3, 6, 192, 192},
                              {3, 7, 192, 256}, {3, 7, 256, 192},
                              {3, 8, 256, 256}};
  for (const Row& r : gains)
    if (r.k == k && r.rate == rate && r.cin == cin && r.cout == cout) return 7;
  return 0;
}

int conv_image_tiles_g(int B, int S, int k, int rate, int cin, int cout) {
  const int g = g_conv_image_tiles < 0 ? conv_image_tiles_rule(k, rate, cin, cout, B, S) : g_conv_image_tiles;
  if (g < 4 || g > 7 || k < 2 || cin < BK || cin % BK || g_conv_variant == 0) return 0;
  if (B % (1 << g) || S % (128 >> g)) return 0;
  return g;
}

inline int image_tile_taps(int mt, int S, int k, int rate, int pad, int g) {
  int y, x0, ul, uh, vl, vh;
  image_tile_pos(mt, S, g, y, x0);
  live_taps_image_tile(y, x0, 128 >> g, S, k, rate, pad, ul, uh, vl, vh);
  return (uh - ul) * (vh - vl);
}

std::vector<int> conv_image_order(int B, int S, int k, int rate, int pad, int g) {
  const int mt = B * S * S / 128;
  std::vector<int> taps(mt), sorted(mt), order(mt);
  for (int i = 0; i < mt; ++i) taps[i] = image_tile_taps(i, S, k, rate, pad, g);
  std::iota(sorted.begin(), sorted.end(), 0);
  std::stable_sort(sorted.begin(), sorted.end(), [&](int x, int y) { return taps[x] > taps[y]; });
  if (mt % 8) return sorted;
  const int per = mt / 8;
  for (int c = 0; c < 8; ++c)
    for (int j = 0; j < per; ++j) order[c * per + j] = sorted[j * 8 + c];
  return order;
}

const int* conv_image_order_device(int B, int S, int k, int rate, int pad, int g) {
  static std::mutex mu;
  static std::map<std::tuple<int, int, int, int, int, int, int>, const int*> cache;
  int dev = 0;
  if (hipGetDevice(&dev) != hipSuccess) return nullptr;
  std::lock_guard<std::mutex> lock(mu);
  const auto key = std::make_tuple(dev, B, S, k, rate, pad, g);
  const auto it = cache.find(key);
  if (it != cache.end()) return it->second;
  const std::vector<int> order = conv_image_order(B, S, k, rate, pad, g);
  int* d = nullptr;
  if (hipMalloc((void**)&d, order.size() * sizeof(int)) != hipSuccess) return nullptr;
  if (hipMemcpy(d, order.data(), order.size() * sizeof(int), hipMemcpyHostToDevice) != hipSuccess) { (void)hipFree(d); return nullptr; }
  cache[key] = d;
  return d;
}

template <int BM, int BN, int WM, int WN>
int launch_conv_dma(ConvArgs& a, float* ws, size_t ws_floats, hipStream_t st) {
  const int mt = (a.M + BM - 1) / BM, nt = a.Cout / BN;
  const int nks = a.k * a.k * (a.Cin / BK);
  const SkGeom g = ws && (reinterpret_cast<uintptr_t>(ws) & 15) == 0 ? sk_geometry(mt * nt, nks, BN, ws_floats) : SkGeom{0, 0, 0};
  const int W = g.W;
  a.sk_W = W; a.sk_nks = nks; a.sk_U = g.T * nks; a.sk_slab = ws;
  a.sk_T = g.T; a.sk_tiles = mt * nt; a.sk_G = g.G; a.sk_order = g_conv_sk_order;
  a.prio = g_conv_prio >= 0 ? g_conv_prio : (g.G && (long long)mt * nt * nks >= 20LL * g.G ? 1 : 0);
  if (g_conv_prio < 0 && drs_chain_level(drs_tl_chain, drs_g_chain_mode) >= 1) a.prio = 3;
  conv_lpt_setup(a, BM, mt, nt, g.G);
  if (!g.G && !a.stats) {
    const int B = a.M / (a.S * a.S);
    a.img_g = conv_image_tiles_g(B, a.S, a.k, a.rate, a.Cin, a.Cout);
    if (a.img_g) {
      a.img_order = conv_image_order_device(B, a.S, a.k, a.rate, a.pad, a.img_g);
      if (!a.img_order) return DRS_ERR_HIP;
      a.lpt_T = 0;
      a.skip_halo = drs_g_skip_halo_taps != 0;
    }
  }
  if (g.G) DRS_LAUNCH((conv_dma_kernel<BM, BN, WM, WN, true>), dim3(g.G), dim3(256), 0, st, a);
  else DRS_LAUNCH((conv_dma_kernel<BM, BN, WM, WN, false>), dim3(mt * nt), dim3(256), 0, st, a);
  int rc = DRS_LAUNCH_CHECK();
  if (rc || !g.G) return rc;
  if (a.sk_U % W == 0 && (a.sk_U / W) % nks == 0) return rc;
  DRS_LAUNCH((conv_sk_fixup_kernel<BM, BN, WM, WN>), dim3(g.T), dim3(256), 0, st, a);
  return DRS_LAUNCH_CHECK();
}

template <int BM, int BN, int WM, int WN>
int launch_conv(ConvArgs& a, float* ws, size_t ws_floats, hipStream_t st) {
  const int mt = (a.M + BM - 1) / BM, nt = a.Cout / BN;
  if (a.Cin < BK) DRS_LAUNCH((conv_igemm_kernel<BM, BN, WM, WN, true>), dim3(mt * nt), dim3(256), 0, st, a);
  else if constexpr (BM == 128) {
    const bool dma = g_conv_variant != 0;
    if (dma) return launch_conv_dma<BM, BN, WM, WN>(a, ws, ws_floats, st);
    DRS_LAUNCH((conv_igemm_kernel<BM, BN, WM, WN>), dim3(mt * nt), dim3(256), 0, st, a);
  } else DRS_LAUNCH((conv_igemm_kernel<BM, BN, WM, WN>), dim3(mt * nt), dim3(256), 0, st, a);
  return DRS_LAUNCH_CHECK();
}

int g_wgrad_variant = -1;

inline bool wgrad_affine(const WgradArgs& a) { return (a.S & 31) == 0 || a.ablate == 5; }
int g_wgrad_seg = 1;
inline bool wgrad_segments(const WgradArgs& a) {
  const long long Sxp = a.S + 2 * a.Px, Sgp = a.S + 2 * a.Pg, B = a.M / ((long long)a.S * a.S);
  const long long xb = (B * Sxp * Sxp + 64) * a.ld_x * 4, gb = (B * Sgp * Sgp + 64) * a.ld_g * 4;
  return g_wgrad_seg && a.S >= 32 && !wgrad_affine(a) && xb < (1LL << 32) && gb < (1LL << 32);
}

template <int TR, int TO>
int launch_wgrad(const WgradArgs& a, int nwg, hipStream_t st) {
  constexpr int NT = 64 * (TR >= 64 ? 2 : 1) * (TO >= 64 ? 2 : 1);
  const bool dma = g_wgrad_variant < 0 ? (TO == 128 || (TO == 64 && (wgrad_affine(a) || (wgrad_segments(a) && a.M < (1 << 18))))) : g_wgrad_variant == 1;
  if (!dma && wgrad_affine(a)) DRS_LAUNCH((wgrad_kernel<TR, TO, true>), dim3(nwg), dim3(NT), 0, st, a);
  else if (!dma) DRS_LAUNCH((wgrad_kernel<TR, TO, false>), dim3(nwg), dim3(NT), 0, st, a);
  else if (wgrad_affine(a)) DRS_LAUNCH((wgrad_dma_kernel<TR, TO, 1>), dim3(nwg), dim3(NT), 0, st, a);
  else if (wgrad_segments(a)) DRS_LAUNCH((wgrad_dma_kernel<TR, TO, 2>), dim3(nwg), dim3(NT), 0, st, a);
  else DRS_LAUNCH((wgrad_dma_kernel<TR, TO, 0>), dim3(nwg), dim3(NT), 0, st, a);
  return DRS_LAUNCH_CHECK();
}

template <int TR, int TO>
int launch_wgrad_dma_only(const WgradArgs& a, int nwg, hipStream_t st) {
  if (wgrad_affine(a)) DRS_LAUNCH((wgrad_dma_kernel<TR, TO, 1>), dim3(nwg), dim3(256), 0, st, a);
  else if (wgrad_segments(a)) DRS_LAUNCH((wgrad_dma_kernel<TR, TO, 2>), dim3(nwg), dim3(256), 0, st, a);
  else DRS_LAUNCH((wgrad_dma_kernel<TR, TO, 0>), dim3(nwg), dim3(256), 0, st, a);
  return DRS_LAUNCH_CHECK();
}

}

__attribute__((visibility("hidden"))) int drs_step_prep(const StepPrepArgs& a, hipStream_t stream) {
  if (a.n < 0 || a.n > STEP_PREP_MAX) return DRS_ERR_ARG;
  DRS_LAUNCH(step_prep_kernel, dim3(512, a.n + 2), dim3(256), 0, stream, a);
  return DRS_LAUNCH_CHECK();
}


int drs_g_skip_halo_taps = 1;
thread_local int drs_tl_chain = 0;
int drs_g_chain_mode = -1;

namespace {

int g_wgrad_target = 2048;

int pick_tile(int c) { return c % 128 == 0 ? 128 : (c % 64 == 0 ? 64 : 32); }
int g_conv_wide192 = 1;
int pick_conv_tile(int c, int cin) { return (g_conv_wide192 && c % 192 == 0 && c % 128 != 0 && cin % 32 == 0 && g_conv_variant != 0) ? 192 : pick_tile(c); }

int pick_wgrad_rows(int rows) {
  const int n128 = (rows + 127) / 128;
  if ((double)rows / (n128 * 128.0) >= 0.85) return 128;
  if (rows % 64 == 0) return 64;
  return rows % 32 == 0 && rows < 128 ? 32 : 128;
}

int pick_wgrad_cols(int tr, int cout) { return (tr == 128 && cout % 192 == 0 && cout % 128 != 0 && g_wgrad_variant != 0) ? 192 : pick_tile(cout); }

int g_wgrad_balance = 1;
int g_wgrad_len = 0;
inline int wgrad_len(int nchunks) { return g_wgrad_len ? g_wgrad_len : (nchunks >= (1 << 14) ? 192 : 96); }
int g_wgrad_minchunks = 8;
int g_wgrad_target_big = 0;

int g_wgrad_prio = -1;
int g_wgrad_ablate = 0;
int g_wgrad_model = 1;

int wgrad_target(long long work, int ntile, int nchunks, bool balanced, int occ, int len = 0) {
  if (len <= 0) len = wgrad_len(nchunks);
  long long fit = work / len;
  fit = fit < 512 ? 512 : (fit > g_wgrad_target ? g_wgrad_target : fit);
  const bool big = ntile >= 24 && nchunks >= 8192;
  if (!balanced) return big ? 2 * g_wgrad_target : (int)fit;
  if (big) return g_wgrad_target_big ? g_wgrad_target_big : 3 * 1024;
  if (g_wgrad_model) {
    static const double eff[5] = {1.0, 0.75, 0.88, 0.93, 0.95};
    const double W0 = (double)work / (double)cu_count(), o = 6.0;
    int n = 1;
    double bt = 1e30;
    for (int i = 1; i <= occ && i <= 4; ++i) {
      const double t = (W0 + i * o) / eff[i];
      if (t < bt) { bt = t; n = i; }
    }
    int r = (int)(W0 / n / (double)len + 0.5);
    r = r < 1 ? 1 : r;
    const long long t = (long long)cu_count() * n * r;
    return (int)(t > 4096 ? 4096 : t);
  }
  static const int steps[] = {512, 768, 1024, 2048, 3072, 4096};
  int best = steps[0];
  for (int s : steps)
    if (s <= g_wgrad_target && (double)(s > fit ? s : fit) / (s > fit ? fit : s) < (double)(best > fit ? best : fit) / (best > fit ? fit : best)) best = s;
  return best;
}

int wgrad_uniform_splits(int B, int S, int k, int cin, int cout, int len = 0) {
  const long long M = (long long)B * S * S;
  const int tr = pick_wgrad_rows(k * k * cin), to = pick_wgrad_cols(tr, cout);
  const int ntile = ((k * k * cin + tr - 1) / tr) * (cout / to);
  const int nchunks = (int)((M + 31) / 32);
  int want = wgrad_target((long long)nchunks * ntile, ntile, nchunks, false, 4, len) / ntile;
  int maxs = (nchunks + g_wgrad_minchunks - 1) / g_wgrad_minchunks;
  if (maxs < 1) maxs = 1;
  if (want > maxs) want = maxs;
  if (want < 1) want = 1;
  const int cps = (nchunks + want - 1) / want;
  return (nchunks + cps - 1) / cps;
}

bool wgrad_live_plan(int B, int S, int k, int rate, int pad, int cin, int cout, int tr, int to, int cap, WgradPlan& p, int& nwg) {
  const int rows = k * k * cin, ntr = (rows + tr - 1) / tr, nto = cout / to;
  p.nclass = 0;
  if (ntr > WG_MAXT) return false;
  int lp[WG_MAXT], vals[WG_MAXC], nv = 0;
  for (int r = 0; r < ntr; ++r) {
    int lo, hi;
    const int rlast = ((r + 1) * tr < rows ? (r + 1) * tr : rows) - 1;
    live_pixel_range(r * tr, rlast, cin, k, rate, pad, S, 1, lo, hi);
    lp[r] = hi - lo;
    int c = 0;
    while (c < nv && vals[c] != lp[r]) ++c;
    if (c == nv) { if (nv == WG_MAXC) return false; vals[nv++] = lp[r]; }
  }
  if (nv == 1 && vals[0] == S * S) return false;
  for (int i = 1; i < nv; ++i)
    for (int j = i; j > 0 && vals[j] < vals[j - 1]; --j) { const int t = vals[j]; vals[j] = vals[j - 1]; vals[j - 1] = t; }
  int cnt[WG_MAXC] = {0};
  for (int r = 0; r < ntr; ++r) {
    int c = 0;
    while (vals[c] != lp[r]) ++c;
    p.cls[r] = (unsigned char)c;
    ++cnt[c];
  }
  const long long M = (long long)B * S * S;
  const int nchunks = (int)((M + 31) / 32);
  double work = 0;
  for (int c = 0; c < nv; ++c) work += (double)cnt[c] * nto * B * vals[c] / 32.0;
  const int target = wgrad_target((long long)work, ntr * nto, nchunks, true, (tr == 128 && to == 192) ? 3 : 4);
  const double len = work / target;
  int maxs = (nchunks + g_wgrad_minchunks - 1) / g_wgrad_minchunks;
  if (maxs > cap) maxs = cap;
  if (maxs < 1) maxs = 1;
  double frac[WG_MAXC];
  int total = 0;
  for (int c = 0; c < nv; ++c) {
    const double x = (double)B * vals[c] / 32.0 / len;
    int n = (int)x;
    frac[c] = x - n;
    if (n > maxs) { n = maxs; frac[c] = 0; }
    if (n < 1) { n = 1; frac[c] = 0; }
    p.n[c] = n;
    total += n * cnt[c] * nto;
  }
  for (;;) {
    int pick = -1;
    for (int c = 0; c < nv; ++c)
      if (frac[c] > 0 && p.n[c] < maxs && total + cnt[c] * nto <= target && (c + 1 == nv || p.n[c] < p.n[c + 1]) && (pick < 0 || frac[c] > frac[pick])) pick = c;
    if (pick < 0) break;
    ++p.n[pick];
    total += cnt[pick] * nto;
    frac[pick] = 0;
  }
  for (int c = 1; c < nv; ++c)
    if (p.n[c] < p.n[c - 1]) p.n[c] = p.n[c - 1];
  int above = ntr, start = 0;
  for (int j = 0; j < nv; ++j) {
    p.seg_start[j] = start;
    p.seg_width[j] = above * nto;
    start += (p.n[j] - (j ? p.n[j - 1] : 0)) * above * nto;
    above -= cnt[j];
  }
  p.seg_start[nv] = start;
  p.nclass = nv;
  nwg = start;
  return true;
}

int wgrad_bound_splits(int B, int S, int k, int cin, int cout) {
  const int shortest = g_wgrad_len && g_wgrad_len < 96 ? g_wgrad_len : 96;
  const int ua = wgrad_uniform_splits(B, S, k, cin, cout), ub = wgrad_uniform_splits(B, S, k, cin, cout, shortest);
  const int u = ua > ub ? ua : ub;
  int maxs = (int)(((long long)B * S * S + 32LL * g_wgrad_minchunks - 1) / (32LL * g_wgrad_minchunks));
  if (maxs < 1) maxs = 1;
  const int bound = u + u / 2 + 1;
  return bound < maxs ? bound : (maxs > u ? maxs : u);
}

int wgrad_setup(int B, int S, int k, int rate, int pad_before, int cin, int cout, WgradArgs& a, int& nwg, int& tr, int& to, int& nsplit) {
  if ((cin % 32 && cin != 8 && cin != 16) || cout % 32 || B < 1 || S < 1 || k < 1 || rate < 1) return DRS_ERR_ARG;
  const long long M = (long long)B * S * S;
  if (M <= 0 || M >= (1 << 24)) return DRS_ERR_ARG;
  a.x = nullptr; a.g = nullptr; a.slab = nullptr; a.Px = a.Pg = a.ld_x = a.ld_g = a.coff_x = a.coff_g = 0;
  a.S = S; a.M = (int)M;
  a.k = k; a.rate = rate; a.pad = pad_before; a.Cin = cin; a.Cout = cout;
  tr = pick_wgrad_rows(k * k * cin); to = pick_wgrad_cols(tr, cout);
  a.ntr = (k * k * cin + tr - 1) / tr; a.nto = cout / to;
  nsplit = wgrad_uniform_splits(B, S, k, cin, cout);
  const int nchunks = (int)((M + 31) / 32);
  a.chunks_per_split = (nchunks + nsplit - 1) / nsplit;
  a.rcpS = 1.0f / (float)S; a.rcpSS = 1.0f / (float)(S * S);
  a.ablate = g_wgrad_ablate;
  a.prio = g_wgrad_prio >= 0 ? g_wgrad_prio : ((g_wgrad_ablate != 3 && M >= (1LL << 18)) ? 1 : 0);
#ifdef DRS_DEV
  a.trace = g_conv_trace;
#endif
  nwg = nsplit * a.ntr * a.nto;
  a.plan.nclass = 0;
  a.live_cut = 0;
  if (g_wgrad_balance && wgrad_live_plan(B, S, k, rate, pad_before, cin, cout, tr, to, wgrad_bound_splits(B, S, k, cin, cout), a.plan, nwg)) {
    a.live_cut = 1;
    a.skip_halo = drs_g_skip_halo_taps != 0;
  } else {
    a.skip_halo = drs_skip_halo_taps_wgrad(M);
    a.live_cut = a.skip_halo;
  }
  return DRS_OK;
}

int conv_plain_image_g(int B, int S, int k, int rate, int cin, int cout) {
  if (cin < 32 || cin % 32) return 0;
  const int bn = pick_conv_tile(cout, cin);
  if (bn < 64) return 0;
  const int mt = (int)(((long long)B * S * S + 127) / 128), nt = cout / bn;
  if (sk_geometry(mt * nt, k * k * (cin / 32), bn, 2ull * (size_t)sk_max_w() * 128 * (size_t)bn).G) return 0;
  return conv_image_tiles_g(B, S, k, rate, cin, cout);
}

}

extern "C" {

#ifdef DRS_DEV
int drs_debug_skip_taps(int v) { const int old = drs_g_skip_halo_taps; if (v >= 0) drs_g_skip_halo_taps = v; return old; }

int drs_debug_wgrad_target(int v) { const int old = g_wgrad_target; if (v > 0) g_wgrad_target = v; return old; }

int drs_debug_wgrad_balance(int v) { const int old = g_wgrad_balance; if (v >= 0) g_wgrad_balance = v; return old; }

int drs_debug_wgrad_len(int v) { const int old = g_wgrad_len; if (v >= 0) g_wgrad_len = v; return old; }

int drs_debug_wgrad_minchunks(int v) { const int old = g_wgrad_minchunks; if (v > 0) g_wgrad_minchunks = v; return old; }

int drs_debug_wgrad_model(int v) { const int old = g_wgrad_model; if (v >= 0) g_wgrad_model = v; return old; }

int drs_debug_wgrad_prio(int v) { const int old = g_wgrad_prio; if (v >= -1) g_wgrad_prio = v; return old; }

int drs_debug_wgrad_ablate(int v) { const int old = g_wgrad_ablate; if (v >= 0) g_wgrad_ablate = v; return old; }

int drs_debug_wgrad_target_big(int v) { const int old = g_wgrad_target_big; if (v >= 0) g_wgrad_target_big = v; return old; }

int drs_debug_conv_wide192(int v) { const int old = g_conv_wide192; if (v >= 0) g_conv_wide192 = v; return old; }

int drs_debug_conv_variant(int v) { const int old = g_conv_variant; if (v >= -1) g_conv_variant = v; return old; }

size_t drs_conv_workspace_floats(int cout);
int drs_debug_conv_lpt(int v) { const int old = g_conv_lpt; if (v >= 0) g_conv_lpt = v; return old; }
int drs_debug_conv_order(int B, int S, int k, int rate, int pad_before, int cin, int cout, int* out, int cap) {
  const long long M = (long long)B * S * S;
  if (M <= 0 || M >= (1 << 24) || cout % 32 || k < 1 || rate < 1) return -1;
  ConvArgs a;
  a.S = S; a.M = (int)M; a.k = k; a.rate = rate; a.pad = pad_before; a.Cin = cin; a.Cout = cout;
  a.skip_halo = drs_skip_halo_taps_fwd(M, cout);
  const int bn = pick_conv_tile(cout, cin);
  if (bn < 64) return 0;
  const int mt = (int)((M + 127) / 128), nt = cout / bn;
  const int W = cin >= 32 ? sk_geometry(mt * nt, k * k * (cin / 32), bn, drs_conv_workspace_floats(cout)).G : 0;
  conv_lpt_setup(a, 128, mt, nt, W);
  if (!a.lpt_T) return 0;
  for (int w = 0; w < mt * nt && w < cap; ++w) out[w] = lpt_tile(w, a.lpt_T, a.lpt_ta, a.lpt_tb, a.lpt_P, nt);
  return mt * nt;
}
int drs_debug_conv_image_tiles(int g) { const int old = g_conv_image_tiles; if (g >= -1) g_conv_image_tiles = g; return old; }
int drs_debug_conv_order_image(int B, int S, int k, int rate, int pad_before, int cin, int cout, int* out, int cap) {
  const long long M = (long long)B * S * S;
  if (M <= 0 || M >= (1 << 24) || cout % 32 || k < 1 || rate < 1) return -1;
  const int g = conv_plain_image_g(B, S, k, rate, cin, cout);
  if (!g) return 0;
  const int mt = (int)(M / 128), nt = cout / pick_conv_tile(cout, cin);
  const std::vector<int> order = conv_image_order(B, S, k, rate, pad_before, g);
  for (int w = 0; w < mt * nt && w < cap; ++w) out[w] = order[w / nt] * nt + w % nt;
  return mt * nt;
}
int drs_debug_conv_trace(void* dev_buffer) { g_conv_trace = (unsigned long long*)dev_buffer; return 0; }

int drs_debug_conv_splitk(int v) { const int old = g_conv_splitk; if (v >= -1) g_conv_splitk = v; return old; }
int drs_debug_conv_hybrid(int v) { const int old = g_conv_hybrid; if (v >= 0) g_conv_hybrid = v; return old; }
int drs_debug_conv_sk_order(int v) { const int old = g_conv_sk_order; if (v >= 0) g_conv_sk_order = v; return old; }
int drs_debug_chain_mode(int v) { const int old = drs_g_chain_mode; if (v >= -1) drs_g_chain_mode = v; return old; }
int drs_debug_conv_prio(int v) { const int old = g_conv_prio; if (v >= -1) g_conv_prio = v; return old; }
int drs_debug_conv_sk_geometry(int tiles, int nks, int bn, int* out3) {
  const SkGeom g = sk_geometry(tiles, nks, bn, 2ull * (size_t)sk_max_w() * 128 * (size_t)bn);
  if (out3) { out3[0] = g.G; out3[1] = g.W; out3[2] = g.T; }
  return g.G;
}

int drs_debug_wgrad_variant(int v) { const int old = g_wgrad_variant; if (v >= -1) g_wgrad_variant = v; return old; }
int drs_debug_wgrad_seg(int v) { const int old = g_wgrad_seg; if (v >= 0) g_wgrad_seg = v; return old; }

#endif

int drs_conv_mtile(int cout) { return pick_tile(cout) >= 64 ? 128 : 256; }

size_t drs_conv_workspace_floats(int cout) {
  const int bn = pick_conv_tile(cout, 32);
  return bn >= 64 ? 2ull * (size_t)sk_max_w() * 128 * (size_t)bn : 0;
}

int drs_conv_halo_skip(int B, int S, int k, int rate, int pad_before, int cin, int cout) {
  const long long M = (long long)B * S * S;
  if (M <= 0 || M >= (1 << 24) || cout % 32 || cin < 32 || cin % 32 || k < 1 || rate < 1) return 0;
  ConvArgs a;
  a.S = S; a.M = (int)M; a.k = k; a.rate = rate; a.pad = pad_before; a.Cin = cin; a.Cout = cout;
  a.skip_halo = drs_skip_halo_taps_fwd(M, cout);
  const int bn = pick_conv_tile(cout, cin);
  if (bn < 64) return a.skip_halo;
  const int mt = (int)((M + 127) / 128), nt = cout / bn;
  const int W = sk_geometry(mt * nt, k * k * (cin / 32), bn, drs_conv_workspace_floats(cout)).G;
  if (W) return 0;
  conv_lpt_setup(a, 128, mt, nt, 0);
  return a.skip_halo;
}

int drs_conv_executed_ksteps(int B, int S, int k, int rate, int pad_before, int cin, int cout, long long* executed, long long* total) {
  const long long M = (long long)B * S * S;
  if (M <= 0 || M >= (1 << 24) || cout % 32 || cin < 1 || k < 1 || rate < 1 || !executed || !total) return DRS_ERR_ARG;
  const int bn = pick_conv_tile(cout, cin), bm = bn >= 64 ? 128 : 256;
  const int mt = (int)((M + bm - 1) / bm), nt = cout / bn;
  const long long cpt = cin < 32 ? 1 : cin / 32;
  *total = *executed = cin < 32 ? (long long)mt * nt * ((k * k * cin + 31) / 32) : (long long)mt * nt * k * k * cpt;
  if (cin < 32 || cin % 32) return DRS_OK;
  const int g = conv_plain_image_g(B, S, k, rate, cin, cout);
  long long taps = 0;
  if (g) {
    if (drs_g_skip_halo_taps == 0) return DRS_OK;
    for (int i = 0; i < mt; ++i) taps += image_tile_taps(i, S, k, rate, pad_before, g);
  } else {
    if (!drs_conv_halo_skip(B, S, k, rate, pad_before, cin, cout)) return DRS_OK;
    for (int i = 0; i < mt; ++i) {
      const int p0 = i * bm, p1 = (int)(p0 + bm < M ? p0 + bm : M) - 1;
      int y0 = (p0 % (S * S)) / S, y1 = (p1 % (S * S)) / S;
      if (p0 / (S * S) != p1 / (S * S)) { y0 = 0; y1 = S - 1; }
      int lo = pad_before - y1 > 0 ? (pad_before - y1 + rate - 1) / rate : 0, hi = (S - 1 - y0 + pad_before) / rate + 1;
      hi = hi < k ? hi : k;
      if (lo >= hi) { lo = 0; hi = k; }
      taps += (hi - lo) * k;
    }
  }
  *executed = taps * nt * cpt;
  return DRS_OK;
}

int drs_conv_forward_ws(const float* in, int B, int S, int P, int ld_in, int coff_in, const float* w, const float* bias,
                        int k, int rate, int pad_before, int cin, int cout, float* out, int ld_out, int coff_out,
                        int accumulate, float* stats_partial, float* workspace, size_t workspace_floats, void* stream) {
  if (!in || !w || !out || (cin % 32 && cin != 8 && cin != 16) || cout % 32 || k < 1 || rate < 1 || P < pad_before) return DRS_ERR_ARG;
  if (cin < 32 && (ld_in % 4 || coff_in % 4)) return DRS_ERR_ARG;
  if (accumulate && stats_partial) return DRS_ERR_ARG;
  if (P < (k - 1) * rate - pad_before) return DRS_ERR_ARG;
  const long long M = (long long)B * S * S;
  if (M <= 0 || M >= (1 << 24)) return DRS_ERR_ARG;
  if ((long long)B * (S + 2 * P) * (S + 2 * P) * ld_in >= (1LL << 30)) return DRS_ERR_ARG;
  ConvArgs a;
  a.in = in; a.S = S; a.P = P; a.ld_in = ld_in; a.coff_in = coff_in; a.M = (int)M;
  a.w = w; a.bias = bias; a.out = out; a.ld_out = ld_out; a.coff_out = coff_out; a.stats = stats_partial;
  a.k = k; a.rate = rate; a.pad = pad_before; a.Cin = cin; a.Cout = cout; a.accumulate = accumulate;
  a.rcpS = 1.0f / (float)S; a.rcpSS = 1.0f / (float)(S * S);
  a.skip_halo = drs_skip_halo_taps_fwd(M, cout);
  a.sk_slab = nullptr; a.sk_W = 0; a.sk_nks = 0; a.sk_U = 0; a.sk_T = a.sk_tiles = a.sk_G = a.sk_order = 0; a.prio = 0;
  a.lpt_T = a.lpt_ta = a.lpt_tb = a.lpt_P = 0;
  a.img_g = 0; a.img_order = nullptr;
#ifdef DRS_DEV
  a.trace = g_conv_trace;
#endif
  hipStream_t st = (hipStream_t)stream;
  if (!workspace) workspace_floats = 0;
  switch (pick_conv_tile(cout, cin)) {
    case 192: return launch_conv_dma<128, 192, 2, 2>(a, workspace, workspace_floats, st);
    case 128: return launch_conv<128, 128, 2, 2>(a, workspace, workspace_floats, st);
    case 64:  return launch_conv<128, 64, 2, 2>(a, workspace, workspace_floats, st);
    default:  return launch_conv<256, 32, 4, 1>(a, workspace, workspace_floats, st);
  }
}

int drs_conv_forward(const float* in, int B, int S, int P, int ld_in, int coff_in, const float* w, const float* bias,
                     int k, int rate, int pad_before, int cin, int cout, float* out, int ld_out, int coff_out,
                     int accumulate, float* stats_partial, void* stream) {
  return drs_conv_forward_ws(in, B, S, P, ld_in, coff_in, w, bias, k, rate, pad_before, cin, cout, out, ld_out, coff_out, accumulate,
                             stats_partial, nullptr, 0, stream);
}

int drs_conv_wgrad_splits(int B, int S, int k, int cin, int cout) { return wgrad_bound_splits(B, S, k, cin, cout); }

#ifdef DRS_DEV
int drs_debug_wgrad_cut(int B, int S, int k, int rate, int pad_before, int cin, int cout, int* out, int cap, int* out_tile_splits,
                        int* out_tile_rows) {
  WgradArgs a;
  int nwg, tr, to, nsplit;
  if (wgrad_setup(B, S, k, rate, pad_before, cin, cout, a, nwg, tr, to, nsplit)) return -1;
  if (out_tile_rows) *out_tile_rows = tr;
  for (int r = 0; r < a.ntr && out_tile_splits; ++r) out_tile_splits[r] = a.plan.nclass ? a.plan.n[a.plan.cls[r]] : nsplit;
  for (int i = 0; i < nwg && i < cap && out; ++i) {
    int tile, split, cbeg, cend, lo, hi;
    wgrad_assign(a, tr, i, tile, split, cbeg, cend, lo, hi);
    out[5 * i] = tile / a.nto; out[5 * i + 1] = tile % a.nto; out[5 * i + 2] = split; out[5 * i + 3] = cbeg; out[5 * i + 4] = cend;
  }
  return nwg;
}
#endif

int drs_conv_wgrad(const float* x, int B, int S, int Px, int ld_x, int coff_x, const float* g, int Pg, int ld_g,
                   int coff_g, int k, int rate, int pad_before, int cin, int cin_real, int cout, float* slab,
                   float* grad, void* stream) {
  if (!x || !g || !slab || !grad || cin_real > cin) return DRS_ERR_ARG;
  if ((long long)B * (S + 2 * Px) * (S + 2 * Px) * ld_x >= (1LL << 30)) return DRS_ERR_ARG;
  if ((long long)B * (S + 2 * Pg) * (S + 2 * Pg) * ld_g >= (1LL << 30)) return DRS_ERR_ARG;
  WgradArgs a;
  int nwg, tr, to, nsplit;
  if (wgrad_setup(B, S, k, rate, pad_before, cin, cout, a, nwg, tr, to, nsplit)) return DRS_ERR_ARG;
  a.x = x; a.Px = Px; a.ld_x = ld_x; a.coff_x = coff_x;
  a.g = g; a.Pg = Pg; a.ld_g = ld_g; a.coff_g = coff_g; a.slab = slab;
  hipStream_t st = (hipStream_t)stream;
  int rc;
  if (tr == 128 && to == 192) rc = launch_wgrad_dma_only<128, 192>(a, nwg, st);
  else if (tr == 128 && to == 128) rc = launch_wgrad<128, 128>(a, nwg, st);
  else if (tr == 128 && to == 64) rc = launch_wgrad<128, 64>(a, nwg, st);
  else if (tr == 128 && to == 32) rc = launch_wgrad<128, 32>(a, nwg, st);
  else if (tr == 64 && to == 128) rc = launch_wgrad<64, 128>(a, nwg, st);
  else if (tr == 64 && to == 64) rc = launch_wgrad<64, 64>(a, nwg, st);
  else if (tr == 64 && to == 32) rc = launch_wgrad<64, 32>(a, nwg, st);
  else if (tr == 32 && to == 128) rc = launch_wgrad<32, 128>(a, nwg, st);
  else if (tr == 32 && to == 64) rc = launch_wgrad<32, 64>(a, nwg, st);
  else rc = launch_wgrad<32, 32>(a, nwg, st);
  if (rc) return rc;
  const int n = k * k * cin_real * cout;
  DRS_LAUNCH(wgrad_reduce_kernel, dim3((n + 255) / 256 < 2048 ? (n + 255) / 256 : 2048), dim3(256), 0, st, slab,
                     grad, nsplit, k * k, cin, cin_real, cout, tr, a.plan);
  return DRS_LAUNCH_CHECK();
}

int drs_filter_flip_transpose(const float* w, float* wt, int k, int cin, int cout, void* stream) {
  if (!w || !wt) return DRS_ERR_ARG;
  const int n = k * k * cin * cout;
  DRS_LAUNCH(flip_transpose_kernel, dim3((n + 255) / 256 < 2048 ? (n + 255) / 256 : 2048), dim3(256), 0,
                     (hipStream_t)stream, w, wt, k, cin, cout);
  return DRS_LAUNCH_CHECK();
}

int drs_filter_pad_cin(const float* w, float* wp, int k, int cin, int cin_pad, int cout, void* stream) {
  if (!w || !wp || cin_pad < cin) return DRS_ERR_ARG;
  const int n = k * k * cin_pad * cout;
  DRS_LAUNCH(pad_cin_kernel, dim3((n + 255) / 256 < 2048 ? (n + 255) / 256 : 2048), dim3(256), 0,
                     (hipStream_t)stream, w, wp, k * k, cin, cin_pad, cout);
  return DRS_LAUNCH_CHECK();
}

}
```

dynamic-rs-segmentation_amd/csrc/drs_common.hpp:

```cpp
#pragma once
#include <hip/hip_runtime.h>
#include <stdint.h>

#define DRS_OK 0
#define DRS_ERR_ARG 1
#define DRS_ERR_HIP 2

typedef float f32x4 __attribute__((ext_vector_type(4)));
typedef float f32x16 __attribute__((ext_vector_type(16)));

struct ActView {
  float* base;
  int S;
  int P;
  int ld;
  int coff;
  uint16_t* terms;
  int nt;
};

__device__ __forceinline__ void view_store4(const ActView& v, size_t e, f32x4 x) {
  if (v.base) *reinterpret_cast<f32x4*>(v.base + e) = x;
  if (v.terms) {
    uint16_t* t = v.terms + (e & ~(size_t)31) * v.nt + (e & 31);
    f32x4 r = x;
    for (int s = 0; s < v.nt; ++s) {
      typedef __bf16 bf16x4_t __attribute__((ext_vector_type(4)));
      bf16x4_t h;
#pragma unroll
      for (int j = 0; j < 4; ++j) h[j] = (__bf16)r[j];
#pragma unroll
      for (int j = 0; j < 4; ++j) r[j] -= (float)h[j];
      *reinterpret_cast<bf16x4_t*>(t + 32 * s) = h;
    }
  }
}

__device__ __forceinline__ void divmod24(int n, int d, float rcp, int& q, int& r) {
  q = (int)((float)n * rcp);
  r = n - q * d;
  if (r < 0) { q -= 1; r += d; }
  else if (r >= d) { q += 1; r -= d; }
}

__device__ __forceinline__ uint32_t padded_pixel_off(int p, int S, int P, int ld, float rcpS, float rcpSS, int dy, int dx) {
  int b, rem, y, x;
  divmod24(p, S * S, rcpSS, b, rem);
  divmod24(rem, S, rcpS, y, x);
  const int Sp = S + 2 * P;
  return (uint32_t)(((b * Sp + y + P + dy) * Sp + (x + P + dx))) * (uint32_t)ld;
}

constexpr int STEP_PREP_MAX = 24;
struct StepPrepArgs {
  const float* w[STEP_PREP_MAX];
  float* wt[STEP_PREP_MAX];
  int k[STEP_PREP_MAX], cin[STEP_PREP_MAX], cout[STEP_PREP_MAX];
  int n;
  unsigned int* z0; int nz0;
  float* z1; int nz1;
};

__device__ __forceinline__ void live_tap_rows(int m0, int BM, int M, int S, int k, int rate, int pad, float rcpS, float rcpSS,
                                              int& lo, int& hi) {
  const int p1 = (m0 + BM - 1 < M ? m0 + BM : M) - 1;
  int b0, r0, b1, r1, y0, y1, x;
  divmod24(m0, S * S, rcpSS, b0, r0);
  divmod24(p1, S * S, rcpSS, b1, r1);
  divmod24(r0, S, rcpS, y0, x);
  divmod24(r1, S, rcpS, y1, x);
  if (b0 != b1) { y0 = 0; y1 = S - 1; }
  const int a = pad - y1;
  lo = a > 0 ? (a + rate - 1) / rate : 0;
  const int bnum = S - 1 - y0 + pad;
  hi = bnum / rate + 1;
  hi = hi < k ? hi : k;
  if (lo >= hi) { lo = 0; hi = k; }
}

__host__ __device__ __forceinline__ void live_taps_image_tile(int y, int x0, int Pc, int S, int k, int rate, int pad,
                                                              int& u_lo, int& u_hi, int& v_lo, int& v_hi) {
  const int au = pad - y, av = pad - (x0 + Pc - 1);
  u_lo = au > 0 ? (au + rate - 1) / rate : 0;
  v_lo = av > 0 ? (av + rate - 1) / rate : 0;
  u_hi = (S - 1 - y + pad) / rate + 1;
  v_hi = (S - 1 - x0 + pad) / rate + 1;
  u_hi = u_hi < k ? u_hi : k;
  v_hi = v_hi < k ? v_hi : k;
  if (u_lo >= u_hi || v_lo >= v_hi) { u_lo = v_lo = 0; u_hi = v_hi = k; }
}
__host__ __device__ __forceinline__ int image_tile_pos(int mt, int S, int g, int& y, int& x0) {
  const int Pc = 128 >> g, npc = S / Pc;
  const int t2 = mt / npc;
  x0 = (mt - t2 * npc) * Pc;
  const int grp = t2 / S;
  y = t2 - grp * S;
  return grp;
}

__host__ __device__ __forceinline__ void live_pixel_range(int row_first, int row_last, int Cin, int k, int rate, int pad, int S, int enable,
                                                          int& lo, int& hi) {
  const int dy_min = (row_first / Cin / k) * rate - pad, dy_max = (row_last / Cin / k) * rate - pad;
  int ylo = -dy_max > 0 ? -dy_max : 0;
  int yhi = S - dy_min < S ? S - dy_min : S;
  if (!enable || ylo >= yhi) { ylo = 0; yhi = S; }
  lo = ylo * S;
  hi = yhi * S;
}

__device__ __forceinline__ int next_live_chunk(int c, int S2, float rcpSS, int lo, int hi) {
  const int p = 32 * (c + 1);
  int b, r;
  divmod24(p, S2, rcpSS, b, r);
  if (r + 31 >= lo && r < hi) return c + 1;
  if (r + 31 >= S2 + lo) return c + 1;
  return ((r < lo ? b : b + 1) * S2 + lo) >> 5;
}

template <int NSLOT, int WM, int BN, class Col, class LaneSum, class Each>
__device__ __forceinline__ void tile_column_stats(float* red, int t, int wm, bool writer, float n_tile, Col col, LaneSum lanesum,
                                                  Each each, float* dst) {
  float* red2 = red + WM * BN;
#pragma unroll
  for (int ni = 0; ni < NSLOT; ++ni) {
    float s = 0.f;
    each(ni, [&](float v) { s += v; });
    s = lanesum(s);
    if (writer) red[wm * BN + col(ni)] = s;
  }
  __syncthreads();
  const float rn = 1.0f / n_tile;
#pragma unroll
  for (int ni = 0; ni < NSLOT; ++ni) {
    float tot = 0.f;
#pragma unroll
    for (int w = 0; w < WM; ++w) tot += red[w * BN + col(ni)];
    const float mean = tot * rn;
    float q = 0.f;
    each(ni, [&](float v) { const float d = v - mean; q += d * d; });
    q = lanesum(q);
    if (writer) red2[wm * BN + col(ni)] = q;
  }
  __syncthreads();
  if (t >= 0 && t < BN && dst) {
    float u1 = 0.f, u2 = 0.f;
#pragma unroll
    for (int w = 0; w < WM; ++w) { u1 += red[w * BN + t]; u2 += red2[w * BN + t]; }
    dst[2 * t] = u1;
    dst[2 * t + 1] = u2;
  }
}

inline int drs_chain_level(int asked, int mode) { return asked == 0 ? 0 : (mode < 0 ? asked : mode); }
extern thread_local int drs_tl_chain;
extern int drs_g_chain_mode;

extern int drs_g_skip_halo_taps;
static inline int drs_skip_halo_taps_fwd(long long M, int cout) {
  if (drs_g_skip_halo_taps != 1) return drs_g_skip_halo_taps == 2;
  const long long wgs = ((M + 127) / 128) * ((cout + 127) / 128);
  return wgs >= 4096;
}
static inline int drs_skip_halo_taps_wgrad(long long M) {
  if (drs_g_skip_halo_taps != 1) return drs_g_skip_halo_taps == 2;
  return M >= (1LL << 19);
}

__device__ __forceinline__ int xcd_remap(int bid, int nblk) {
  const int xcd = bid & 7, q = nblk >> 3, r = nblk & 7;
  const int start = xcd < r ? xcd * (q + 1) : r * (q + 1) + (xcd - r) * q;
  return start + (bid >> 3);
}

static inline int drs_check(hipError_t e) { return e == hipSuccess ? DRS_OK : DRS_ERR_HIP; }
#define DRS_LAUNCH_CHECK() drs_check(hipGetLastError())
#define DRS_LAUNCH(...) do { (void)hipGetLastError(); hipLaunchKernelGGL(__VA_ARGS__); } while (0)
```

include/drs.h:

```cpp
#ifndef DRS_H_
#define DRS_H_
#include <stddef.h>

#ifdef __cplusplus
extern "C" {
#endif

#define DRS_OK 0
#define DRS_ERR_ARG 1
#define DRS_ERR_HIP 2

int drs_conv_mtile(int cout);
size_t drs_conv_workspace_floats(int cout);
int drs_conv_halo_skip(int B, int S, int k, int rate, int pad_before, int cin, int cout);
int drs_conv_executed_ksteps(int B, int S, int k, int rate, int pad_before, int cin, int cout, long long* executed, long long* total);
int drs_conv_forward_ws(const float* in, int B, int S, int P, int ld_in, int coff_in, const float* w, const float* bias,
                        int k, int rate, int pad_before, int cin, int cout, float* out, int ld_out, int coff_out,
                        int accumulate, float* stats_partial, float* workspace, size_t workspace_floats, void* stream);
int drs_conv_forward(const float* in, int B, int S, int P, int ld_in, int coff_in, const float* w, const float* bias,
                     int k, int rate, int pad_before, int cin, int cout, float* out, int ld_out, int coff_out,
                     int accumulate, float* stats_partial, void* stream);

int drs_conv_wgrad_splits(int B, int S, int k, int cin, int cout);
int drs_conv_wgrad(const float* x, int B, int S, int Px, int ld_x, int coff_x, const float* g, int Pg, int ld_g,
                   int coff_g, int k, int rate, int pad_before, int cin, int cin_real, int cout, float* slab,
                   float* grad, void* stream);

int drs_filter_flip_transpose(const float* w, float* wt, int k, int cin, int cout, void* stream);
int drs_filter_pad_cin(const float* w, float* wp, int k, int cin, int cin_pad, int cout, void* stream);

int drs_split_conv_mtile(int cout);
int drs_split_terms(const float* src, size_t n, int nterms, unsigned short* terms, void* stream);
int drs_filter_split(const float* w, int k, int cin, int cin_pad, int cout, int nterms, unsigned short* wf,
                     unsigned short* wd, void* stream);
int drs_conv_forward_split(const unsigned short* in, int B, int S, int P, int ld_in, int coff_in, const unsigned short* w,
                           const float* bias, int k, int rate, int pad_before, int cin, int cout, float* out, int ld_out,
                           int coff_out, int accumulate, float* stats_partial, int nterms, void* stream);
int drs_conv_wgrad_split_splits(int B, int S, int k, int cin, int cout, int Pg, int nterms);
int drs_conv_wgrad_split(const unsigned short* x, int B, int S, int Px, int ld_x, int coff_x, const unsigned short* g,
                         int Pg, int ld_g, int coff_g, int k, int rate, int pad_before, int cin, int cin_real, int cout,
                         float* slab, float* grad, int nterms, void* stream);

int drs_colsum_scratch_doubles(int ncols);
int drs_stats_reduce(const float* partial, int nrows, int C, double* sums, double* scratch, void* stream);
int drs_stats_reduce_means(const float* partial, int nrows, int C, double count, double* sums, float* means, void* stream);
int drs_conv_stats_reduce(const float* partial, int M, int mtile, int C, double* sums, double* scratch, void* stream);
int drs_conv_stats_finish(const float* partial, int M, int mtile, int C, double count, float* mean_rstd, float* moving_mean,
                          float* moving_var, double decay, int bessel, double* sums, void* stream);
int drs_bn_finish(const double* sums, double count, int C, float* mean_rstd, float* moving_mean, float* moving_var,
                  double decay, int bessel, void* stream);
int drs_bn_eval_coeffs(const float* moving_mean, const float* moving_var, int C, float* mean_rstd, void* stream);

int drs_bn_act_pool_forward(const float* z, int B, int S, int C, const float* mean_rstd, float alpha, int pool,
                            float* out, int P_out, int ld_out, int coff_out, unsigned char* argmax, void* stream);
int drs_bn_finish_act_pool_forward(const double* sums, double count, float* mean_rstd, float* moving_mean, float* moving_var, double decay,
                                   int bessel_moving_var, const float* z, int B, int S, int C, float alpha, int pool, float* out, int P_out,
                                   int ld_out, int coff_out, unsigned char* argmax, void* stream);
int drs_bn_act_pool_forward_terms(const float* z, int B, int S, int C, const float* mean_rstd, float alpha, int pool,
                                  float* out, int P_out, int ld_out, int coff_out, unsigned char* argmax,
                                  unsigned short* terms, int nterms, void* stream);

int drs_bn_backward_rows(int B, int S, int C, int pool);
int drs_bn_backward_reduce(const float* ga, int ld_ga, int coff_ga, const float* z, const unsigned char* argmax, int B,
                           int S, int C, const float* mean_rstd, float alpha, int pool, float* gxhat, float* partial,
                           void* stream);
int drs_bn_backward_apply(const float* gxhat, const float* z, int B, int S, int C, const float* mean_rstd,
                          const double* sums, double count, float* gz, int P_out, int ld_out, int coff_out,
                          void* stream);
int drs_bn_backward_apply_means(const float* gxhat, const float* z, int B, int S, int C, const float* mean_rstd,
                                const float* means, float* gz, int P_out, int ld_out, int coff_out, void* stream);
int drs_bn_backward_apply_terms(const float* gxhat, const float* z, int B, int S, int C, const float* mean_rstd,
                                const double* sums, double count, float* gz, int P_out, int ld_out, int coff_out,
                                unsigned short* terms, int nterms, void* stream);

int drs_avg_pool_forward(const float* in, int B, int S, int C, int k, float* out, int P_out, int ld_out, int coff_out,
                         void* stream);
int drs_avg_pool_backward(const float* gout, int ld_g, int coff_g, int B, int S, int C, int k, float* gin, void* stream);

int drs_se_forward(const float* act, int B, int S, int C, int R, const float* w1, const float* b1, const float* w2, const float* b2,
                   float* s, float* e1, float* e2, float* out, int P_out, int ld_out, int coff_out, void* stream);
int drs_se_backward(const float* gy, int ld_g, int coff_g, const float* act, const float* s, const float* e1, const float* e2,
                    const float* w1, const float* w2, int B, int S, int C, int R, float* gact, float* dw1, float* db1, float* dw2,
                    float* db2, float* scratch, void* stream);
int drs_se_core_sums_scratch_doubles(int C);
int drs_se_core_sums(const float* act, int C, int T, const int* boxes, int n, double* sums, double* scratch, void* stream);
int drs_se_gate(const double* sums, double count, int C, int R, const float* w1, const float* b1, const float* w2, const float* b2,
                float* s, float* e1, float* e2, void* stream);
int drs_se_scale_const(const float* act, int B, int S, int C, const float* e2, float* out, int P_out, int ld_out, int coff_out,
                       void* stream);

int drs_classifier_rows(int B, int S);
int drs_classifier_loss(const float* feat, int B, int S, int P, int ld, int coff, int C, int K, const float* w,
                        const float* bias, const unsigned char* labels, const unsigned char* loss_mask,
                        const unsigned char* acc_mask, float inv_n, float* logits, unsigned char* pred, float* gfeat,
                        int ld_g, int coff_g, float* dw_partial, float* db_partial, double* loss_partial,
                        unsigned int* conf, void* stream);
int drs_classifier_loss_weighted(const float* feat, int B, int S, int P, int ld, int coff, int C, int K, const float* w,
                                 const float* bias, const unsigned char* labels, const unsigned char* loss_mask,
                                 const unsigned char* acc_mask, float inv_n, const float* class_weights, float* logits,
                                 unsigned char* pred, float* gfeat, int ld_g, int coff_g, float* dw_partial, float* db_partial,
                                 double* loss_partial, unsigned int* conf, void* stream);
int drs_classifier_loss_focal(const float* feat, int B, int S, int P, int ld, int coff, int C, int K, const float* w,
                              const float* bias, const unsigned char* labels, const unsigned char* loss_mask,
                              const unsigned char* acc_mask, float inv_n, const float* class_weights, float focal_gamma,
                              float* logits, unsigned char* pred, float* gfeat, int ld_g, int coff_g, float* dw_partial,
                              float* db_partial, double* loss_partial, unsigned int* conf, void* stream);
int drs_label_histogram(const unsigned char* labels, size_t n, int K, int void_label, unsigned long long* counts, void* stream);
int drs_reliability_histogram(const unsigned char* truth, const unsigned char* pred, const unsigned char* confidence, size_t n, int K,
                              int ignore_label, unsigned long long* hist, void* stream);
size_t drs_temperature_scratch_doubles(size_t n);
int drs_temperature_stats(const float* sums, const unsigned int* occur, const unsigned char* truth, size_t n, int K, int sums_are_prob,
                          int ignore_label, double beta, double* scratch, double* out , void* stream);

int drs_rows_reduce_f32(const float* in, int nrows, int ncols, float* out, double* scratch, void* stream);
int drs_sum_f64(const double* in, int n, double* out, void* stream);
int drs_scale_f64(double* x, int n, double s, void* stream);
int drs_l2_loss(const float* w, size_t n, double* scratch, double* out, void* stream);

int drs_momentum_update(float* w, const float* grad, float* accum, size_t n, size_t n_decay, float lr,
                        float weight_decay, float momentum, float grad_scale, void* stream);

int drs_confusion(const unsigned char* labels, const unsigned char* pred, const unsigned char* mask, size_t n, int K,
                  int ignore_label, unsigned int* conf, void* stream);

int drs_crop_normalize(const void* tiles, int tiles_are_f64, const unsigned char* labels, const long long* tile_off,
                       const long long* lab_off, const int* tile_h, const int* tile_w, int C, const int* inst,
                       const double* rot, const unsigned char* rot_on, const double* noise,
                       const unsigned char* noise_on, unsigned long long seed, int noise_index0, const double* mean3,
                       const double* std3,
                       int B, int S, int P, int ld, float* out, unsigned char* out_lab, unsigned char* out_mask,
                       int void_label, int quantize_f16, void* stream);
int drs_crop_normalize_scaled(const void* tiles, int tiles_are_f64, const unsigned char* labels, const long long* tile_off,
                              const long long* lab_off, const int* tile_h, const int* tile_w, int n_maps, int C, const int* inst,
                              const double* geo, const double* rot, const unsigned char* rot_on, const double* noise,
                              const unsigned char* noise_on, unsigned long long seed, int noise_index0, const double* mean3,
                              const double* std3, int B, int S, int P, int ld, float* out, unsigned char* out_lab,
                              unsigned char* out_mask, int void_label, int quantize_f16, void* stream);

int drs_stitch_accumulate(float* prob, unsigned int* occur, const float* logits, int h, int w, int K, int S, int stride,
                          int first_window, int n_windows, void* stream);
int drs_stitch_finalize(const float* prob, const unsigned int* occur, int h, int w, int K, unsigned char* out,
                        void* stream);
int drs_tile_place(float* prob, unsigned int* occur, const float* logits, int h, int w, int K, int T, const int* boxes, int n,
                   void* stream);
int drs_crop_dihedral(const void* tiles, int tiles_are_f64, const long long* tile_off, const int* tile_h, const int* tile_w, int n_maps,
                      int C, const int* inst, int g, const double* mean3, const double* std3, int B, int T, int P, int ld, float* out,
                      void* stream);
int drs_tile_place_dihedral(float* acc, unsigned int* occur, const float* logits, int h, int w, int K, int T, const int* boxes, int n,
                            int g, void* stream);
int drs_crop_resampled(const void* tiles, int tiles_are_f64, const long long* tile_off, const int* tile_h, const int* tile_w, int n_maps,
                       int C, const int* inst, int hs, int ws, int g, const double* mean3, const double* std3, int B, int T, int P, int ld,
                       float* out, void* stream);
int drs_resample_accumulate(const float* src, const unsigned int* occur, int hs, int ws, int K, int src_is_prob, int h, int w, float* acc,
                            void* stream);
int drs_stitch_finalize_scores(const float* sums, const unsigned int* occur, int h, int w, int K, int sums_are_prob,
                               unsigned char* labels, unsigned char* confidence, unsigned char* margin, unsigned char* entropy,
                               void* stream);
int drs_stitch_finalize_scores_t(const float* sums, const unsigned int* occur, int h, int w, int K, int sums_are_prob, float beta,
                                 unsigned char* labels, unsigned char* confidence, unsigned char* margin, unsigned char* entropy,
                                 void* stream);
int drs_softmax_accumulate(const float* prob, const unsigned int* occur, int h, int w, int K, float* acc, void* stream);

typedef struct drs_net drs_net_t;
typedef int (*drs_allreduce_fn)(void* user, void* dev_ptr, size_t count, int dtype, int async, void* stream);
typedef int (*drs_wait_fn)(void* user, int handle, void* stream);
#define DRS_WANT_LOGITS 1
#define DRS_WITH_LABELS 2
#define DRS_USE_ACC_MASK 4
#define DRS_USE_LOSS_MASK 8
#define DRS_NO_UPDATE 16

int drs_net_create(const char* net_type, int channels, int num_classes, float weight_decay, int b_max, int s_max, int bessel_moving_var,
                   float lr_decay_factor, drs_net_t** out);
void drs_net_destroy(drs_net_t* net);
int drs_net_num_buffers(const drs_net_t* net);
int drs_net_buffer_info(const drs_net_t* net, int index, char* name, int name_cap, size_t* bytes, int* dtype);
int drs_net_bind(drs_net_t* net, const char* name, void* dev_ptr, size_t bytes);
int drs_net_buffer(drs_net_t* net, const char* name, void** dev_ptr, size_t* bytes);
int drs_net_layout(const drs_net_t* net, size_t* n_params, size_t* n_decay, size_t* n_bn, int* n_layers, int* x0_channels, int* x0_halo);
int drs_net_layer_info(const drs_net_t* net, int index, char* name, int name_cap, int* geom8, char* src_slab, char* dst_slab, int slab_cap,
                       int* dst_coff, int* pool);
int drs_net_info(const drs_net_t* net, char* net_type, int name_cap, float* alpha, int* c_last, char* feat_slab, int slab_cap, int* topology,
                 int* n_se);
int drs_net_receptive_field(const drs_net_t* net, int* before, int* after);
int drs_net_receptive_field_gated(const drs_net_t* net, int* before, int* after);
int drs_net_se_info(const drs_net_t* net, int index, char* scope, int scope_cap, int* layer, int* channels, int* reduced);
int drs_net_type_name(int index, char* name, int name_cap, int* canonical);
int drs_net_num_variables(const drs_net_t* net);
int drs_net_variable_info(const drs_net_t* net, int index, char* name, int name_cap, size_t* offset, size_t* count, int* shape4, int* in_bn);
int drs_params_get(drs_net_t* net, const char* name, const char* slot, float* host_dst, size_t count, void* stream);
int drs_params_set(drs_net_t* net, const char* name, const char* slot, const float* host_src, size_t count, void* stream);
int drs_grad_buffer(drs_net_t* net, float** dev_ptr, size_t* count);
long long drs_net_global_step(drs_net_t* net, long long set_to);
float drs_net_learning_rate(const drs_net_t* net, float lr0);
int drs_net_set_comm(drs_net_t* net, int world, int rank, drs_allreduce_fn allreduce, drs_wait_fn wait, void* user);
#define DRS_RCCL_FORM_INLINE 1
#define DRS_RCCL_FORM_ASYNC 2
#define DRS_RCCL_FORM_BUCKETS 3
int drs_rccl_form(void);
int drs_rccl_bind_library(const char* path);
int drs_rccl_available(void);
int drs_rccl_unique_id(unsigned char* id128);
int drs_rccl_comm_create(int world, int rank, const unsigned char* id128, void** comm);
int drs_rccl_comm_destroy(void* comm);
int drs_rccl_all_reduce(void* comm, void* dev_ptr, size_t count, int dtype, void* stream);
int drs_net_set_rccl(drs_net_t* net, int world, int rank, void* comm_small, void* comm_big, void* comm_stream);
int drs_train_step(drs_net_t* net, int B, int S, float lr0, int flags, double global_pixels, void* stream);
int drs_forward(drs_net_t* net, int B, int S, int flags, int ignore_label, void* stream);
int drs_apply_update(drs_net_t* net, float lr0, void* stream);
int drs_forward_staged(drs_net_t* net, int B, int S, int stage, const int* boxes, int n_boxes, int flags, void* stream);
int drs_net_se_gate_finish(drs_net_t* net, int index, double count, void* stream);
int drs_net_set_two_streams(drs_net_t* net, int mode);
int drs_net_set_class_weights(drs_net_t* net, const float* host_w, int K);
int drs_net_get_class_weights(const drs_net_t* net, float* host_w, int K_cap, int* is_set);
int drs_net_set_focal_gamma(drs_net_t* net, float gamma);
int drs_net_get_focal_gamma(const drs_net_t* net, float* gamma);
int drs_net_timing(drs_net_t* net, int enable);
int drs_net_num_timing_kinds(void);
int drs_net_timing_summary(drs_net_t* net, int kind, char* name, int name_cap, int* launches, double* ms, double* work);

#ifdef __cplusplus
}
#endif
#endif
```

include/drs_dev.h:

```cpp
#ifndef DRS_DEV_H_
#define DRS_DEV_H_
#ifdef __cplusplus
extern "C" {
#endif

int drs_debug_skip_taps(int v);
int drs_debug_conv_variant(int v);
int drs_debug_conv_wide192(int v);
int drs_debug_conv_lpt(int v);
int drs_debug_conv_order(int B, int S, int k, int rate, int pad_before, int cin, int cout, int* out, int cap);
int drs_debug_conv_image_tiles(int g);
int drs_debug_conv_order_image(int B, int S, int k, int rate, int pad_before, int cin, int cout, int* out, int cap);
int drs_debug_conv_trace(void* dev_buffer);
int drs_debug_conv_splitk(int v);
int drs_debug_conv_hybrid(int v);
int drs_debug_conv_sk_order(int v);
int drs_debug_conv_prio(int v);
int drs_debug_conv_sk_geometry(int tiles, int nks, int bn, int* out3);
int drs_debug_wgrad_variant(int v);
int drs_debug_wgrad_seg(int v);
int drs_debug_wgrad_balance(int v);
int drs_debug_wgrad_target(int v);
int drs_debug_wgrad_target_big(int v);
int drs_debug_wgrad_len(int v);
int drs_debug_wgrad_minchunks(int v);
int drs_debug_wgrad_prio(int v);
int drs_debug_wgrad_ablate(int v);
int drs_debug_wgrad_model(int v);
int drs_debug_slide_blocks(int v);
int drs_debug_slide_minrows(int v);
int drs_debug_jitter(unsigned long long seed);
int drs_debug_wg_stream_prio(int arm);
int drs_debug_reductions_on_chain(int on);
int drs_debug_wgrad_schedule(int layer_slabs, int streams, int defer);
int drs_debug_chain_mode(int v);
int drs_debug_slide_rowpad(int v);
int drs_debug_cls_variant(int v);
int drs_debug_variant(int v);
int drs_debug_wgrad_cut(int B, int S, int k, int rate, int pad_before, int cin, int cout, int* out, int cap, int* out_tile_splits,
                        int* out_tile_rows);

#ifdef __cplusplus
}
#endif
#endif
```

Baseline: 2719 patches/s.

## Add 2D live-pixel window walk to wgrad DMA kernel for dilated halo skipping

Adds a window-walk mode to the weight-gradient DMA kernel. For each row tile it computes the live pixel rectangle (both y and x bounds) for the dilated taps and walks only pixels inside it, so columns that only touch padding halo are skipped rather than just whole rows. The mode is enabled by default for the 3x3 rate-8 256->256 layer at batch 128 and 64x64, and adds per-chunk jump/valid-count bookkeeping, tail zeroing and a reworked priority schedule. The gain depends on how much column halo is removed versus the cost of extra segment handling and partially filled chunks.

```diff
diff --git a/dynamic-rs-segmentation_amd/_lib.py b/dynamic-rs-segmentation_amd/_lib.py
--- a/dynamic-rs-segmentation_amd/_lib.py
+++ b/dynamic-rs-segmentation_amd/_lib.py
@@ -14,6 +14,7 @@
     "drs_conv_workspace_floats": (_sz, [_i]),
     "drs_conv_halo_skip": (_i, [_i, _i, _i, _i, _i, _i, _i]),
     "drs_conv_executed_ksteps": (_i, [_i, _i, _i, _i, _i, _i, _i, _p, _p]),
+    "drs_wgrad_executed_chunks": (_i, [_i, _i, _i, _i, _i, _i, _i, _p, _p]),
     "drs_conv_forward_ws": (_i, [_p, _i, _i, _i, _i, _i, _p, _p, _i, _i, _i, _i, _i, _p, _i, _i, _i, _p, _p, _sz, _p]),
     "drs_conv_wgrad_splits": (_i, [_i, _i, _i, _i, _i]),
     "drs_conv_wgrad": (_i, [_p, _i, _i, _i, _i, _i, _p, _i, _i, _i, _i, _i, _i, _i, _i, _i, _p, _p, _p]),
@@ -135,6 +136,7 @@
     "drs_debug_wgrad_variant": (_i, [_i]), "drs_debug_wgrad_seg": (_i, [_i]), "drs_debug_wgrad_balance": (_i, [_i]), "drs_debug_wgrad_target": (_i, [_i]),
     "drs_debug_wgrad_target_big": (_i, [_i]), "drs_debug_wgrad_len": (_i, [_i]), "drs_debug_wgrad_minchunks": (_i, [_i]), "drs_debug_wgrad_model": (_i, [_i]), "drs_debug_wgrad_ablate": (_i, [_i]), "drs_debug_wgrad_prio": (_i, [_i]), "drs_debug_cls_variant": (_i, [_i]), "drs_debug_slide_blocks": (_i, [_i]), "drs_debug_slide_minrows": (_i, [_i]), "drs_debug_slide_rowpad": (_i, [_i]), "drs_debug_chain_mode": (_i, [_i]), "drs_debug_jitter": (_i, [C.c_ulonglong]), "drs_debug_wg_stream_prio": (_i, [_i]), "drs_debug_reductions_on_chain": (_i, [_i]), "drs_debug_wgrad_schedule": (_i, [_i, _i, _i]), "drs_debug_variant": (_i, [_i]),
     "drs_debug_wgrad_cut": (_i, [_i] * 7 + [_p, _i, _p, _p]),
+    "drs_debug_wgrad_window": (_i, [_i]), "drs_debug_wgrad_walk": (_i, [_i] * 12 + [_p, _i, _p]),
 }
 
 
diff --git a/dynamic-rs-segmentation_amd/csrc/conv_mfma.hip b/dynamic-rs-segmentation_amd/csrc/conv_mfma.hip
--- a/dynamic-rs-segmentation_amd/csrc/conv_mfma.hip
+++ b/dynamic-rs-segmentation_amd/csrc/conv_mfma.hip
@@ -35,6 +35,12 @@
 #endif
 };
 
+__device__ __forceinline__ void set_prio_level(int level) {
+  if (level >= 3) __builtin_amdgcn_s_setprio(3);
+  else if (level == 2) __builtin_amdgcn_s_setprio(2);
+  else if (level == 1) __builtin_amdgcn_s_setprio(1);
+  else __builtin_amdgcn_s_setprio(0);
+}
 __device__ __forceinline__ void set_prio_by_progress(int done, int total, int& quarter, int mode = 1) {
   const int q = __builtin_amdgcn_readfirstlane((done * 4) / total);
   if (q == quarter) return;
@@ -564,14 +570,6 @@
   unsigned long long* trace;
 #endif
 };
-
-__host__ __device__ __forceinline__ int wave_uniform(int v) {
-#if defined(__HIP_DEVICE_COMPILE__)
-  return __builtin_amdgcn_readfirstlane(v);
-#else
-  return v;
-#endif
-}
 
 __host__ __device__ __forceinline__ void wgrad_assign(const WgradArgs& a, int TR, int id, int& tile, int& split, int& cbeg, int& cend,
                                                       int& live_lo, int& live_hi) {
@@ -658,6 +656,15 @@
     return c - c_old;
   }
 };
+
+__host__ __device__ __forceinline__ int32_t window_jump(const WindowWalk& w, int P, int ld) {
+  if (w.b2 >= w.B) return -(int32_t)((uint32_t)(32 * ld) * 4u);
+  const int Sp = w.S + 2 * P;
+  return (int32_t)((uint32_t)((Sp - (w.xhi - w.xlo) + (w.wrap ? Sp * (Sp - (w.yhi - w.ylo)) : 0)) * ld) * 4u);
+}
+
+template <bool WIN> struct WgradWalk { typedef ChunkWalk type; };
+template <> struct WgradWalk<true> { typedef WindowWalk type; };
 
 template <int TR, int TO, bool AFF>
 __global__ __launch_bounds__(64 * (TR >= 64 ? 2 : 1) * (TO >= 64 ? 2 : 1), 3) void wgrad_kernel(const WgradArgs a) {
@@ -883,8 +890,9 @@
 
   constexpr bool AFF = MODE == 1;
   constexpr bool SEG = MODE == 2;
+  constexpr bool WIN = MODE == 3;
   const int t = threadIdx.x;
-  const int lane = t & 63, wave = (AFF || SEG) ? __builtin_amdgcn_readfirstlane(t >> 6) : t >> 6;
+  const int lane = t & 63, wave = (AFF || SEG || WIN) ? __builtin_amdgcn_readfirstlane(t >> 6) : t >> 6;
   const int li = lane & 31, h = lane >> 5;
   const int wr = wave / WC, wc = wave % WC;
 
@@ -900,13 +908,13 @@
   const int o0 = (tile % a.nto) * TO;
   const int rows_all = a.k * a.k * a.Cin;
   const int Sxp = a.S + 2 * a.Px, Sgp = a.S + 2 * a.Pg;
-  constexpr bool affine = AFF || SEG;
+  constexpr bool affine = AFF || SEG || WIN;
   const int xq = lane % XQ;
   const int myR = R0 + xq * 4;
   const int myRc = myR < rows_all ? myR : 0;
   const int tap = myRc / a.Cin, c0 = myRc % a.Cin;
   const int u = tap / a.k, v = tap % a.k;
-  const uint32_t biasx = SEG ? (uint32_t)(32 * a.ld_x) * 4u : 0u, biasg = SEG ? (uint32_t)(32 * a.ld_g) * 4u : 0u;
+  const uint32_t biasx = (SEG || WIN) ? (uint32_t)(32 * a.ld_x) * 4u : 0u, biasg = (SEG || WIN) ? (uint32_t)(32 * a.ld_g) * 4u : 0u;
   const uint32_t xconst = (uint32_t)((a.ablate == 1 ? 0 : (u * a.rate * Sxp + v * a.rate)) * a.ld_x + a.coff_x + c0) * 4u + biasx;
   uint32_t xoff[IX], goff[IG];
   int xpix[IX], gpix[IG];
@@ -932,8 +940,14 @@
 
   const int nchunks_total = (a.M + BP - 1) / BP;
   const int clast = (a.M & 31) ? nchunks_total - 1 : -1;
-  ChunkWalk w;
-  w.init(cbeg, a.S, a.rcpS, a.rcpSS, live_lo, live_hi);
+  typename WgradWalk<WIN>::type w;
+  int wylo = 0, wyhi = a.S, wxlo = 0, wxhi = a.S;
+  if constexpr (WIN) {
+    const int rlast = (R0 + TR < rows_all ? R0 + TR : rows_all) - 1;
+    live_pixel_window(R0, rlast, a.Cin, a.k, a.rate, a.pad, a.S, a.skip_halo, wylo, wyhi, wxlo, wxhi);
+    if (a.ablate == 6) { wxlo = 0; wxhi = a.S; }
+    w.init(cbeg, cend, a.S, a.M, wylo, wyhi, wxlo, wxhi);
+  } else w.init(cbeg, a.S, a.rcpS, a.rcpSS, live_lo, live_hi);
 
   int py = 0, px = 0;
   uint32_t ox = 0, og = 0;
@@ -970,7 +984,7 @@
   const char* xbase = reinterpret_cast<const char*>(a.x);
   const char* gbase = reinterpret_cast<const char*>(a.g);
   typedef __attribute__((address_space(3))) void* lds_ptr;
-  struct Seg { int brk; int32_t jx, jg; };
+  struct Seg { int brk; int32_t jx, jg; int nv; };
   auto chunk_bases = [&](const char*& xb, const char*& gb, Seg& sg) {
     xb = xbase + (size_t)(uint32_t)(((w.b * Sxp + w.y + a.Px - a.pad) * Sxp + w.x0 + a.Px - a.pad) * a.ld_x) * 4u;
     gb = gbase + (size_t)(uint32_t)(((w.b * Sgp + w.y + a.Pg) * Sgp + w.x0 + a.Pg) * a.ld_g) * 4u;
@@ -981,6 +995,13 @@
       sg.jx = last ? -(int32_t)biasx : (int32_t)(rowjx + (img_end ? imgjx : 0u));
       sg.jg = last ? -(int32_t)biasg : (int32_t)(rowjg + (img_end ? imgjg : 0u));
     }
+    if constexpr (WIN) {
+      xb -= biasx; gb -= biasg;
+      sg.brk = w.brk;
+      sg.nv = w.nv;
+      sg.jx = window_jump(w, a.Px, a.ld_x);
+      sg.jg = window_jump(w, a.Pg, a.ld_g);
+    }
   };
   struct LaneOffsets { uint32_t x[2][IX], g[2][IG]; };
   auto fetch_offsets = [&](int slot, LaneOffsets& o) {
@@ -1000,12 +1021,12 @@
       const char* xh = xb + (size_t)(uint32_t)(half * HP * a.ld_x) * 4u;
       const char* gh = gb + (size_t)(uint32_t)(half * HP * a.ld_g) * 4u;
       int inner = HP;
-      if (SEG) {
+      if (SEG || WIN) {
         const int hb = seg.brk - half * HP;
         if (hb <= 0) { xh += (ptrdiff_t)seg.jx; gh += (ptrdiff_t)seg.jg; }
         else if (hb < HP) inner = hb;
       }
-      if (SEG && inner < HP) {
+      if ((SEG || WIN) && inner < HP) {
 #pragma unroll
         for (int i = 0; i < IX; ++i) {
           uint32_t v = xoff[i] + (xpix[i] >= inner ? (uint32_t)seg.jx : 0u);
@@ -1035,9 +1056,16 @@
       for (int i = 0; i < IG; ++i) __builtin_amdgcn_global_load_lds(gbase + o.g[half][i], (lds_ptr)(sg + (wave + NW * i) * 256), 16, 0, 0);
     }
   };
-  auto zero_tail = [&](int chunk, int half, int stage) {
+  auto zero_tail = [&](int chunk, const Seg& seg, int half, int stage) {
+    float* sg = lds + stage * STAGE + XSTAGE;
+    if constexpr (WIN) {
+      if (seg.nv >= half * HP + HP) return;
+      for (int e = t; e < HP * TO; e += NT)
+        if (half * HP + e / TO >= seg.nv) sg[e] = 0.f;
+      __syncthreads();
+      return;
+    }
     if (AFF || chunk != clast) return;
-    float* sg = lds + stage * STAGE + XSTAGE;
     for (int e = t; e < HP * TO; e += NT)
       if (chunk * BP + half * HP + e / TO >= a.M) sg[e] = 0.f;
     __syncthreads();
@@ -1081,7 +1109,7 @@
 #pragma unroll
       for (int i = 0; i < IG; ++i) oA.g[half][i] = oB.g[half][i] = 0u;
     }
-    Seg sgA = {32, 0, 0}, sgB = {32, 0, 0};
+    Seg sgA = {32, 0, 0, 32}, sgB = {32, 0, 0, 32};
     chunk_bases(xbA, gbA, sgA);
     fill_tables(0, 0);
     if (!affine) __syncthreads();
@@ -1093,9 +1121,18 @@
     fill_tables(1, stepped);
     asm volatile("s_waitcnt vmcnt(0)" ::: "memory");
     __syncthreads();
-    zero_tail(cA, 0, 0);
+    zero_tail(cA, sgA, 0, 0);
     int quart = -1;
+    const int plen = cend - cbeg, pq1 = cbeg + (plen + 3) / 4, pq2 = cbeg + (2 * plen + 3) / 4, pq3 = cbeg + (3 * plen + 3) / 4;
+    int pnext = a.prio ? cbeg : 0x7fffffff;
     for (int it = 0; cA < cend; ++it) {
+      if constexpr (WIN) {
+        while (cA >= pnext) {
+          ++quart;
+          pnext = quart == 0 ? pq1 : (quart == 1 ? pq2 : (quart == 2 ? pq3 : 0x7fffffff));
+          set_prio_level(a.prio == 2 ? (quart < 2 ? 2 - quart : 0) : 3 - quart);
+        }
+      } else
       if (a.prio) set_prio_by_progress(cA - cbeg, cend - cbeg, quart, a.prio);
 #ifdef DRS_DEV
       const bool late = a.ablate == 2;
@@ -1103,10 +1140,11 @@
 #endif
       fetch_offsets((it + 1) & 1, oB);
       issue(xbA, gbA, sgA, oA, 1, 1);
+      if constexpr (WIN) chunk_bases(xbB, gbB, sgB);
       compute(0);
       asm volatile("s_waitcnt vmcnt(0)" ::: "memory");
       __syncthreads();
-      zero_tail(cA, 1, 1);
+      zero_tail(cA, sgA, 1, 1);
 #ifdef DRS_DEV
       if (late) fetch_offsets((it + 1) & 1, oB);
 #endif
@@ -1116,11 +1154,11 @@
       fill_tables(it & 1, stepped);
       asm volatile("s_waitcnt vmcnt(0)" ::: "memory");
       __syncthreads();
-      if (cB < cend) zero_tail(cB, 0, 0);
+      if (cB < cend) zero_tail(cB, sgB, 0, 0);
       cA = cB; xbA = xbB; gbA = gbB; sgA = sgB;
       oA = oB;
       cB = w.c;
-      chunk_bases(xbB, gbB, sgB);
+      if constexpr (!WIN) chunk_bases(xbB, gbB, sgB);
     }
   }
   const size_t rows_total = (size_t)a.k * a.k * a.Cin;
@@ -1404,9 +1442,20 @@
   return g_wgrad_seg && a.S >= 32 && !wgrad_affine(a) && xb < (1LL << 32) && gb < (1LL << 32);
 }
 
+inline bool wgrad_bias_fits(const WgradArgs& a) {
+  const long long Sxp = a.S + 2 * a.Px, Sgp = a.S + 2 * a.Pg, B = a.M / ((long long)a.S * a.S);
+  return (B * Sxp * Sxp + 64) * a.ld_x * 4 < (1LL << 32) && (B * Sgp * Sgp + 64) * a.ld_g * 4 < (1LL << 32);
+}
+
 template <int TR, int TO>
-int launch_wgrad(const WgradArgs& a, int nwg, hipStream_t st) {
+int launch_wgrad(const WgradArgs& a, int nwg, hipStream_t st, bool window = false) {
   constexpr int NT = 64 * (TR >= 64 ? 2 : 1) * (TO >= 64 ? 2 : 1);
+  if constexpr (TR == 128 && (TO == 128 || TO == 64)) {
+    if (window && wgrad_bias_fits(a)) {
+      DRS_LAUNCH((wgrad_dma_kernel<TR, TO, 3>), dim3(nwg), dim3(NT), 0, st, a);
+      return DRS_LAUNCH_CHECK();
+    }
+  }
   const bool dma = g_wgrad_variant < 0 ? (TO == 128 || (TO == 64 && (wgrad_affine(a) || (wgrad_segments(a) && a.M < (1 << 18))))) : g_wgrad_variant == 1;
   if (!dma && wgrad_affine(a)) DRS_LAUNCH((wgrad_kernel<TR, TO, true>), dim3(nwg), dim3(NT), 0, st, a);
   else if (!dma) DRS_LAUNCH((wgrad_kernel<TR, TO, false>), dim3(nwg), dim3(NT), 0, st, a);
@@ -1417,8 +1466,9 @@
 }
 
 template <int TR, int TO>
-int launch_wgrad_dma_only(const WgradArgs& a, int nwg, hipStream_t st) {
-  if (wgrad_affine(a)) DRS_LAUNCH((wgrad_dma_kernel<TR, TO, 1>), dim3(nwg), dim3(256), 0, st, a);
+int launch_wgrad_dma_only(const WgradArgs& a, int nwg, hipStream_t st, bool window = false) {
+  if (window && wgrad_bias_fits(a)) DRS_LAUNCH((wgrad_dma_kernel<TR, TO, 3>), dim3(nwg), dim3(256), 0, st, a);
+  else if (wgrad_affine(a)) DRS_LAUNCH((wgrad_dma_kernel<TR, TO, 1>), dim3(nwg), dim3(256), 0, st, a);
   else if (wgrad_segments(a)) DRS_LAUNCH((wgrad_dma_kernel<TR, TO, 2>), dim3(nwg), dim3(256), 0, st, a);
   else DRS_LAUNCH((wgrad_dma_kernel<TR, TO, 0>), dim3(nwg), dim3(256), 0, st, a);
   return DRS_LAUNCH_CHECK();
@@ -1584,7 +1634,25 @@
   return bound < maxs ? bound : (maxs > u ? maxs : u);
 }
 
-int wgrad_setup(int B, int S, int k, int rate, int pad_before, int cin, int cout, WgradArgs& a, int& nwg, int& tr, int& to, int& nsplit) {
+int g_wgrad_window = -1;
+bool wgrad_window_rule(int k, int rate, int cin, int cout, int B, int S) {
+  return B == 128 && S == 64 && k == 3 && rate == 8 && cin == 256 && cout == 256;
+}
+bool wgrad_window_launch(const WgradArgs& a, int tr, int to, int B) {
+  if (!g_wgrad_window || !a.skip_halo || g_wgrad_variant == 0 || (a.ablate && a.ablate != 6)) return false;
+  if (tr != 128 || (to != 64 && to != 128 && to != 192) || (a.S & 1) || a.S < 32) return false;
+  if (g_wgrad_window < 0 && !wgrad_window_rule(a.k, a.rate, a.Cin, a.Cout, B, a.S)) return false;
+  const int rows = a.k * a.k * a.Cin;
+  for (int r = 0; r < a.ntr; ++r) {
+    int ylo, yhi, xlo, xhi;
+    live_pixel_window(r * tr, ((r + 1) * tr < rows ? (r + 1) * tr : rows) - 1, a.Cin, a.k, a.rate, a.pad, a.S, 1, ylo, yhi, xlo, xhi);
+    if (xhi - xlo < a.S) return true;
+  }
+  return false;
+}
+
+int wgrad_setup(int B, int S, int k, int rate, int pad_before, int cin, int cout, WgradArgs& a, int& nwg, int& tr, int& to, int& nsplit,
+                int* window = nullptr) {
   if ((cin % 32 && cin != 8 && cin != 16) || cout % 32 || B < 1 || S < 1 || k < 1 || rate < 1) return DRS_ERR_ARG;
   const long long M = (long long)B * S * S;
   if (M <= 0 || M >= (1 << 24)) return DRS_ERR_ARG;
@@ -1612,6 +1680,7 @@
     a.skip_halo = drs_skip_halo_taps_wgrad(M);
     a.live_cut = a.skip_halo;
   }
+  if (window) *window = wgrad_window_launch(a, tr, to, B);
   return DRS_OK;
 }
 
@@ -1694,6 +1763,7 @@
 
 int drs_debug_wgrad_variant(int v) { const int old = g_wgrad_variant; if (v >= -1) g_wgrad_variant = v; return old; }
 int drs_debug_wgrad_seg(int v) { const int old = g_wgrad_seg; if (v >= 0) g_wgrad_seg = v; return old; }
+int drs_debug_wgrad_window(int v) { const int old = g_wgrad_window; if (v >= -1) g_wgrad_window = v; return old; }
 
 #endif
 
@@ -1806,6 +1876,95 @@
 }
 #endif
 
+namespace {
+long long wgrad_workgroup_chunks(const WgradArgs& a, int tr, int id, bool window) {
+  int tile, split, cbeg, cend, lo, hi;
+  wgrad_assign(a, tr, id, tile, split, cbeg, cend, lo, hi);
+  long long n = 0;
+  if (window) {
+    const int rows = a.k * a.k * a.Cin, R0 = (tile / a.nto) * tr;
+    int ylo, yhi, xlo, xhi;
+    live_pixel_window(R0, (R0 + tr < rows ? R0 + tr : rows) - 1, a.Cin, a.k, a.rate, a.pad, a.S, a.skip_halo, ylo, yhi, xlo, xhi);
+    if (a.ablate == 6) { xlo = 0; xhi = a.S; }
+    WindowWalk w;
+    w.init(cbeg, cend, a.S, a.M, ylo, yhi, xlo, xhi);
+    for (; w.c < cend; w.advance()) ++n;
+    return n;
+  }
+  const long long S2 = (long long)a.S * a.S;
+  for (long long c = cbeg; c < cend; ++c) {
+    const long long r = (32 * c) % S2;
+    if ((r + 31 >= lo && r < hi) || r + 31 >= S2 + lo) ++n;
+  }
+  return n;
+}
+}
+
+int drs_wgrad_executed_chunks(int B, int S, int k, int rate, int pad_before, int cin, int cout, long long* executed, long long* total) {
+  if (!executed || !total) return DRS_ERR_ARG;
+  WgradArgs a;
+  int nwg, tr, to, nsplit, window;
+  if (wgrad_setup(B, S, k, rate, pad_before, cin, cout, a, nwg, tr, to, nsplit, &window)) return DRS_ERR_ARG;
+  *total = (long long)a.ntr * a.nto * ((a.M + 31) / 32);
+  long long n = 0;
+  for (int i = 0; i < nwg; ++i) n += wgrad_workgroup_chunks(a, tr, i, window != 0);
+  *executed = n;
+  return DRS_OK;
+}
+
+#ifdef DRS_DEV
+int drs_debug_wgrad_walk(int B, int S, int k, int rate, int pad_before, int cin, int cout, int Px, int ld_x, int Pg, int ld_g,
+                         int workgroup, long long* out, int cap, int* info) {
+  WgradArgs a;
+  int nwg, tr, to, nsplit, window;
+  if (wgrad_setup(B, S, k, rate, pad_before, cin, cout, a, nwg, tr, to, nsplit, &window)) return -1;
+  if (workgroup < 0 || workgroup >= nwg || Px < pad_before || Pg < 0) return -1;
+  a.Px = Px; a.ld_x = ld_x; a.Pg = Pg; a.ld_g = ld_g;
+  if (window && !wgrad_bias_fits(a)) window = 0;
+  int tile, split, cbeg, cend, lo, hi;
+  wgrad_assign(a, tr, workgroup, tile, split, cbeg, cend, lo, hi);
+  const int rows = k * k * cin, R0 = (tile / a.nto) * tr;
+  int ylo, yhi, xlo, xhi;
+  live_pixel_window(R0, (R0 + tr < rows ? R0 + tr : rows) - 1, cin, k, rate, pad_before, S, window && a.skip_halo, ylo, yhi, xlo, xhi);
+  if (!window) { ylo = lo / S; yhi = hi / S; xlo = 0; xhi = S; }
+  if (info) { info[0] = window; info[1] = tile / a.nto; info[2] = cbeg; info[3] = cend; info[4] = ylo; info[5] = yhi; info[6] = xlo; info[7] = xhi; }
+  const long long Sxp = S + 2 * Px, Sgp = S + 2 * Pg;
+  auto xo = [&](long long b, long long y, long long x) { return ((b * Sxp + y + Px - pad_before) * Sxp + x + Px - pad_before) * ld_x * 4; };
+  auto go = [&](long long b, long long y, long long x) { return ((b * Sgp + y + Pg) * Sgp + x + Pg) * ld_g * 4; };
+  int n = 0;
+  if (window) {
+    WindowWalk w;
+    w.init(cbeg, cend, S, a.M, ylo, yhi, xlo, xhi);
+    for (; w.c < cend; w.advance(), ++n) {
+      if (n >= cap || !out) continue;
+      const long long jx = window_jump(w, Px, ld_x), jg = window_jump(w, Pg, ld_g);
+      for (int j = 0; j < 32; ++j) {
+        long long* o = out + ((size_t)n * 32 + j) * 3;
+        o[0] = xo(w.b, w.y, w.x0) + (long long)j * ld_x * 4 + (j >= w.brk ? jx : 0);
+        o[1] = go(w.b, w.y, w.x0) + (long long)j * ld_g * 4 + (j >= w.brk ? jg : 0);
+        o[2] = j >= w.nv;
+      }
+    }
+    return n;
+  }
+  const long long S2 = (long long)S * S;
+  for (long long c = cbeg; c < cend; ++c) {
+    const long long r = (32 * c) % S2;
+    if (!((r + 31 >= lo && r < hi) || r + 31 >= S2 + lo)) continue;
+    if (n < cap && out)
+      for (int j = 0; j < 32; ++j) {
+        const long long p = 32 * c + j, q = p < a.M ? p : a.M - 1;
+        long long* o = out + ((size_t)n * 32 + j) * 3;
+        o[0] = xo(q / S2, (q % S2) / S, q % S);
+        o[1] = go(q / S2, (q % S2) / S, q % S);
+        o[2] = p >= a.M;
+      }
+    ++n;
+  }
+  return n;
+}
+#endif
+
 int drs_conv_wgrad(const float* x, int B, int S, int Px, int ld_x, int coff_x, const float* g, int Pg, int ld_g,
                    int coff_g, int k, int rate, int pad_before, int cin, int cin_real, int cout, float* slab,
                    float* grad, void* stream) {
@@ -1813,15 +1972,15 @@
   if ((long long)B * (S + 2 * Px) * (S + 2 * Px) * ld_x >= (1LL << 30)) return DRS_ERR_ARG;
   if ((long long)B * (S + 2 * Pg) * (S + 2 * Pg) * ld_g >= (1LL << 30)) return DRS_ERR_ARG;
   WgradArgs a;
-  int nwg, tr, to, nsplit;
-  if (wgrad_setup(B, S, k, rate, pad_before, cin, cout, a, nwg, tr, to, nsplit)) return DRS_ERR_ARG;
+  int nwg, tr, to, nsplit, window;
+  if (wgrad_setup(B, S, k, rate, pad_before, cin, cout, a, nwg, tr, to, nsplit, &window)) return DRS_ERR_ARG;
   a.x = x; a.Px = Px; a.ld_x = ld_x; a.coff_x = coff_x;
   a.g = g; a.Pg = Pg; a.ld_g = ld_g; a.coff_g = coff_g; a.slab = slab;
   hipStream_t st = (hipStream_t)stream;
   int rc;
-  if (tr == 128 && to == 192) rc = launch_wgrad_dma_only<128, 192>(a, nwg, st);
-  else if (tr == 128 && to == 128) rc = launch_wgrad<128, 128>(a, nwg, st);
-  else if (tr == 128 && to == 64) rc = launch_wgrad<128, 64>(a, nwg, st);
+  if (tr == 128 && to == 192) rc = launch_wgrad_dma_only<128, 192>(a, nwg, st, window);
+  else if (tr == 128 && to == 128) rc = launch_wgrad<128, 128>(a, nwg, st, window);
+  else if (tr == 128 && to == 64) rc = launch_wgrad<128, 64>(a, nwg, st, window);
   else if (tr == 128 && to == 32) rc = launch_wgrad<128, 32>(a, nwg, st);
   else if (tr == 64 && to == 128) rc = launch_wgrad<64, 128>(a, nwg, st);
   else if (tr == 64 && to == 64) rc = launch_wgrad<64, 64>(a, nwg, st);
diff --git a/dynamic-rs-segmentation_amd/csrc/drs_common.hpp b/dynamic-rs-segmentation_amd/csrc/drs_common.hpp
--- a/dynamic-rs-segmentation_amd/csrc/drs_common.hpp
+++ b/dynamic-rs-segmentation_amd/csrc/drs_common.hpp
@@ -108,6 +108,85 @@
   hi = yhi * S;
 }
 
+__host__ __device__ __forceinline__ int wave_uniform(int v) {
+#if defined(__HIP_DEVICE_COMPILE__)
+  return __builtin_amdgcn_readfirstlane(v);
+#else
+  return v;
+#endif
+}
+
+__host__ __device__ __forceinline__ void live_pixel_window(int row_first, int row_last, int Cin, int k, int rate, int pad, int S, int enable,
+                                                           int& ylo, int& yhi, int& xlo, int& xhi) {
+  const int dy_min = (row_first / Cin / k) * rate - pad, dy_max = (row_last / Cin / k) * rate - pad;
+  ylo = -dy_max > 0 ? -dy_max : 0;
+  yhi = S - dy_min < S ? S - dy_min : S;
+  if (!enable || ylo >= yhi) { ylo = 0; yhi = S; }
+  const int t0 = row_first / Cin, t1 = row_last / Cin;
+  int dx_min = (t0 % k) * rate - pad, dx_max = dx_min;
+  for (int t = t0 + 1; t <= t1 && t < t0 + k; ++t) {
+    const int dx = (t % k) * rate - pad;
+    dx_min = dx < dx_min ? dx : dx_min;
+    dx_max = dx > dx_max ? dx : dx_max;
+  }
+  xlo = -dx_max > 0 ? -dx_max : 0;
+  xhi = S - dx_min < S ? S - dx_min : S;
+  xlo &= ~1;
+  xhi = (xhi + 1) & ~1;
+  if (!enable || (S & 1) || xhi - xlo < 32) { xlo = 0; xhi = S; }
+}
+
+struct WindowWalk {
+  int c, b, y, x0, p;
+  int brk, nv, b2, wrap;
+  int S, S2, B, lim, cend_, ylo, yhi, xlo, xhi;
+  int span;
+  __host__ __device__ __forceinline__ void describe() {
+    brk = xhi - x0;
+    wrap = y + 1 == yhi;
+    b2 = b + wrap;
+    nv = 32;
+    if (p + span > lim) {
+      const int p2 = p + brk + (S - (xhi - xlo)) + (wrap ? S2 - (yhi - ylo) * S : 0);
+      const int n1 = brk < 32 ? brk : 32;
+      int v1 = lim - p;
+      v1 = v1 < 0 ? 0 : (v1 < n1 ? v1 : n1);
+      int v2 = 0;
+      if (brk < 32 && v1 == brk && b2 < B) { v2 = lim - p2; v2 = v2 < 0 ? 0 : (v2 < 32 - brk ? v2 : 32 - brk); }
+      nv = wave_uniform(v1 + v2);
+    }
+    c = (b < B && p < lim) ? p >> 5 : cend_;
+  }
+  __host__ __device__ __forceinline__ void init(int cbeg, int cend, int S_, int M, int ylo_, int yhi_, int xlo_, int xhi_) {
+    S = S_; S2 = S_ * S_; B = M / S2; cend_ = cend; ylo = ylo_; yhi = yhi_; xlo = xlo_; xhi = xhi_;
+    lim = 32 * cend < M ? 32 * cend : M;
+    span = 32 + (S - (xhi - xlo)) + (S2 - (yhi - ylo) * S);
+    const int first = 32 * cbeg;
+    b = first / S2;
+    const int r = first - b * S2;
+    y = r / S;
+    x0 = r - y * S;
+    if (x0 >= xhi) { x0 = xlo; ++y; }
+    else if (x0 < xlo) x0 = xlo;
+    if (y < ylo) { y = ylo; x0 = xlo; }
+    else if (y >= yhi) { y = ylo; x0 = xlo; ++b; }
+    p = b * S2 + y * S + x0;
+    describe();
+  }
+  __host__ __device__ __forceinline__ int advance() {
+    if (brk > 32) { x0 += 32; p += 32; }
+    else {
+      const int rem = 32 - brk;
+      p += 32 + (S - (xhi - xlo)) + (wrap ? S2 - (yhi - ylo) * S : 0);
+      x0 = xlo + rem;
+      y = wrap ? ylo : y + 1;
+      b = b2;
+    }
+    describe();
+    return 1;
+  }
+};
+
 __device__ __forceinline__ int next_live_chunk(int c, int S2, float rcpSS, int lo, int hi) {
   const int p = 32 * (c + 1);
   int b, r;
diff --git a/include/drs.h b/include/drs.h
--- a/include/drs.h
+++ b/include/drs.h
@@ -14,6 +14,7 @@
 size_t drs_conv_workspace_floats(int cout);
 int drs_conv_halo_skip(int B, int S, int k, int rate, int pad_before, int cin, int cout);
 int drs_conv_executed_ksteps(int B, int S, int k, int rate, int pad_before, int cin, int cout, long long* executed, long long* total);
+int drs_wgrad_executed_chunks(int B, int S, int k, int rate, int pad_before, int cin, int cout, long long* executed, long long* total);
 int drs_conv_forward_ws(const float* in, int B, int S, int P, int ld_in, int coff_in, const float* w, const float* bias,
                         int k, int rate, int pad_before, int cin, int cout, float* out, int ld_out, int coff_out,
                         int accumulate, float* stats_partial, float* workspace, size_t workspace_floats, void* stream);
diff --git a/include/drs_dev.h b/include/drs_dev.h
--- a/include/drs_dev.h
+++ b/include/drs_dev.h
@@ -19,6 +19,7 @@
 int drs_debug_conv_sk_geometry(int tiles, int nks, int bn, int* out3);
 int drs_debug_wgrad_variant(int v);
 int drs_debug_wgrad_seg(int v);
+int drs_debug_wgrad_window(int v);
 int drs_debug_wgrad_balance(int v);
 int drs_debug_wgrad_target(int v);
 int drs_debug_wgrad_target_big(int v);
@@ -39,6 +40,8 @@
 int drs_debug_variant(int v);
 int drs_debug_wgrad_cut(int B, int S, int k, int rate, int pad_before, int cin, int cout, int* out, int cap, int* out_tile_splits,
                         int* out_tile_rows);
+int drs_debug_wgrad_walk(int B, int S, int k, int rate, int pad_before, int cin, int cout, int Px, int ld_x, int Pg, int ld_g,
+                         int workgroup, long long* out, int cap, int* info);
 
 #ifdef __cplusplus
 }
```

Result: no change. 2717 patches/s (-0.1%).
